# vaenyr/stable-diffusion-on-device

Hardware: AMD Instinct MI355X
Metric: images/sec + per-UNet-step ms, SD v1.4 512x512 20-step PLMS, 1/2/4/8 MI355X (higher is better)
Workload: dtype f16; 1 GPU; SD v1.4 txt2img 512x512, 20-step PLMS (21 UNet evals, batch 2 = cond+uncond per image), CLIP encode + VAE decode + uint8, guidance 7.5; images_per_gpu=1, global_batch=1, parallelism=dp1 (image shards, 1 RCCL broadcast), hip_graph=True, trajectory_graph=True, decode_overlaps_next_sampling=False

## Files before the change

include/sdod_engine.h:

```cpp
#ifndef SDOD_ENGINE_H
#define SDOD_ENGINE_H

#include <stddef.h>
#include <stdint.h>

#ifndef SDOD_API
#define SDOD_API
#endif

#ifdef __cplusplus
extern "C" {
#endif

enum sdod_graph_kind { SDOD_GRAPH_UNET = 0, SDOD_GRAPH_VAE_DECODER = 1, SDOD_GRAPH_TEXT_ENCODER = 2, SDOD_GRAPH_TEMB = 3,
                       SDOD_GRAPH_VAE_ENCODER = 4, SDOD_GRAPH_VAE_ENCODER_MASKED = 5, SDOD_GRAPH_ADAPTER = 6, SDOD_GRAPH_UPSCALER = 7 };

typedef struct sdod_model_config {
    int latent_channels;
    int latent_h;
    int latent_w;
    int model_channels;
    int context_dim;
    int context_len;
    int num_heads;
    int head_dim;
    int vocab_size;
    int text_layers;
    int text_heads;
    int vae_channels;
    int linear_proj;
    int text_arch;
    int weight_quant;
    int concat_channels;
} sdod_model_config;

SDOD_API void sdod_model_config_sd14(sdod_model_config* cfg);
SDOD_API void sdod_model_config_sd21(sdod_model_config* cfg);

SDOD_API int sdod_graph_create(void** graph, int kind, const sdod_model_config* cfg, int batch);
typedef struct sdod_adapter_config {
    int adapter_reps;
    int adapter_hint_channels;
    int adapter_res_blocks;
} sdod_adapter_config;
SDOD_API int sdod_graph_create_ex(void** graph, int kind, const sdod_model_config* cfg, const sdod_adapter_config* adapter, int batch);
SDOD_API int sdod_graph_create_wrap(void** graph, int kind, const sdod_model_config* cfg, const sdod_adapter_config* adapter, int wrap,
                                    int batch);
typedef struct sdod_upscaler_config {
    int num_blocks;
    int in_h;
    int in_w;
} sdod_upscaler_config;
SDOD_API int sdod_graph_create_upscaler(void** graph, const sdod_upscaler_config* cfg, int batch);
SDOD_API int sdod_graph_destroy(void* graph);

SDOD_API int sdod_graph_num_params(void* graph);
SDOD_API int sdod_graph_param_info(void* graph, int index, const char** name, int* ndim, int64_t shape[4]);
SDOD_API int sdod_graph_set_param(void* graph, const char* name, const void* data, int dtype, const int64_t* shape, int ndim);
SDOD_API int sdod_graph_param_device(void* graph, const char* name, void** device_ptr, size_t* bytes);
SDOD_API int sdod_graph_load_file(void* graph, const char* path, const char* prefix);
SDOD_API int sdod_graph_finalize(void* graph);
SDOD_API int sdod_graph_io(void* graph, int is_output, int index, void** device_ptr, size_t* bytes);
enum sdod_exec_flags { SDOD_EXEC_HIP_GRAPH = 1, SDOD_EXEC_STATIC_UNCHANGED = 2 };
SDOD_API int sdod_graph_execute(void* graph, void* stream, int flags);
SDOD_API int sdod_graph_check(void* graph);
SDOD_API int sdod_graph_num_ops(void* graph);
SDOD_API int sdod_graph_op_info(void* graph, int index, const char** label, double* flops, double* bytes);
SDOD_API int sdod_graph_op_detail(void* graph, int index, const char** detail);
SDOD_API int sdod_graph_profile(void* graph, void* stream, int iters, float* ms_out, int n);
SDOD_API int sdod_graph_stats(void* graph, size_t* weight_bytes, size_t* arena_bytes, int* num_launches, double* flops);
SDOD_API int sdod_graph_tune_info(void* graph, int* from_table, int* tuned_in_process, char* table_path, int cap);

SDOD_API int sdod_graph_keep_base(void* graph);
SDOD_API int sdod_graph_base_bytes(void* graph, size_t* bytes);
typedef struct {
    const char* name;
    const void* up;
    const void* down;
    int dtype;
    int rank;
    float scale;
} sdod_lora_entry;
SDOD_API int sdod_graph_set_loras(void* graph, const sdod_lora_entry* entries, int count, void* stream);

#ifdef __cplusplus
}
#endif
#endif
```

include/sdod_hip.h:

```cpp
#ifndef SDOD_HIP_H
#define SDOD_HIP_H

#include <stddef.h>
#include <stdint.h>

#ifndef SDOD_API
#define SDOD_API
#endif

#ifdef __cplusplus
extern "C" {
#endif

enum sdod_act { SDOD_ACT_NONE = 0, SDOD_ACT_SILU = 1, SDOD_ACT_GELU = 2, SDOD_ACT_QUICK_GELU = 3, SDOD_ACT_RELU = 4 };
enum sdod_dtype { SDOD_F16 = 0, SDOD_F32 = 1, SDOD_U8Q = 2, SDOD_BF16 = 3  };
enum sdod_a_mode { SDOD_A_ROWS = 0, SDOD_A_CONV3X3 = 1  };

typedef struct sdod_gemm_desc {
    const void* a;
    const void* a2;
    const void* w;
    const void* bias;
    const void* row_bias;
    const void* residual;
// ... 33 lines not shown
    int vec_img_stride;
    int softmax_cols;
    int pad_mode;
} sdod_gemm_desc;

SDOD_API int sdod_gemm_f16(const sdod_gemm_desc* d, void* stream);
SDOD_API int sdod_gemm_fixup(const sdod_gemm_desc* d);
SDOD_API size_t sdod_gemm_fixup_counters(void);
SDOD_API size_t sdod_gemm_workspace_bytes(const sdod_gemm_desc* d);
SDOD_API int sdod_gemm_plan(const sdod_gemm_desc* d, int* tile, int* splits);
SDOD_API int sdod_gemm_halo_ok(const sdod_gemm_desc* d, int tile);
SDOD_API int sdod_gemm_panel_ok(const sdod_gemm_desc* d, int tile);
SDOD_API int sdod_gemm_xcd_panels(const sdod_gemm_desc* d);
SDOD_API int sdod_gemm_num_tiles(void);
SDOD_API int sdod_gemm_tile_shape(int tile, int* bm, int* bn, int* lds_dma);
SDOD_API int sdod_gemm_tile_info(int tile, int out[7]);
SDOD_API int sdod_gemm_time(const sdod_gemm_desc* d, void* stream, int iters, float* ms_avg);
SDOD_API int sdod_gemm_time_cold(const sdod_gemm_desc* d, void* stream, int iters, void* scratch, size_t scratch_bytes, float* ms_avg,
                                float* ms_min );

SDOD_API size_t sdod_group_norm_workspace_bytes(int n, int groups);
SDOD_API int sdod_group_norm_layout(int n, int groups, size_t* sync_off, size_t* partial_off, size_t* stats_off, size_t* shift_off,
                                    size_t* end_off);
SDOD_API int sdod_group_norm_status(void);
SDOD_API int sdod_group_norm_clear_error(void);
SDOD_API int sdod_group_norm_launches(int hw, int c, int groups, int dtype);
SDOD_API int sdod_group_norm_path(int n, int hw, int c0, int c1, int groups, int dtype);
SDOD_API int sdod_group_norm_nhwc(const void* x, const void* x2, void* y, const float* weight, const float* bias,
                                  int n, int hw, int c0, int c1, int groups, float eps, int silu, int dtype,
                                  void* workspace, void* stream);

SDOD_API size_t sdod_group_norm_nchw_workspace_bytes(int n, int groups);
SDOD_API int sdod_group_norm_nchw(const void* x, void* y, const float* weight, const float* bias, int n, int c, long long spatial,
                                  int groups, float eps, int silu, int dtype, void* workspace, void* stream);

typedef struct sdod_gn_reduce {
    const void* partial;
    int splits;
    size_t slab_floats;
    const void* bias;
    const void* bias2;
    const void* row_bias;
    int ld_row_bias;
    const void* residual;
    int ldr;
    void* x_out;
    float alpha;
    int act;
    int M, N;
} sdod_gn_reduce;
SDOD_API int sdod_gemm_reduce_info(const sdod_gemm_desc* d, sdod_gn_reduce* out);
SDOD_API int sdod_group_norm_reduce_ok(int hw, int c0, int c1, int groups);
SDOD_API int sdod_group_norm_reduce_nhwc(const sdod_gn_reduce* red, const void* x2, void* y, const float* weight,
                                         const float* bias, int n, int hw, int c0, int c1, int groups, float eps, int silu,
                                         void* stream);

SDOD_API int sdod_ln_fold_f16(void* w, int n, int k, int ldw, const float* gamma, const float* beta, const float* bias_in,
                              float* s_out, float* t_out, void* stream);
SDOD_API int sdod_compose_linear_f16(const void* p, int ldp, const void* w, int ldw, void* c, int ldc, int n_out, int n_mid, int k,
                                     const float* bias_w, const float* bias_p, float* bias_out, void* stream);
SDOD_API int sdod_lora_merge_f16(void* w, int n, int k, int ldw, const void* up, const void* down, int rank, float scale,
                                 int conv_cin, int geglu, void* stream);
SDOD_API int sdod_layer_norm_f16(const void* x, void* y, const float* weight, const float* bias, int m, int c,
                                 float eps, void* stream);

SDOD_API int sdod_attention_f16(const void* q, const void* k, const void* v, void* out, int batch, int heads,
                                int lq, int lk, int d, int ldq, int ldk, int ldv, int ldo, float scale, int causal,
                                void* stream);

SDOD_API int sdod_xattn_fold_f16(const void* kv, int ld_kv, int k_off, int v_off, int n_img, int L, const void* wq, int ldq,
                                 const void* sq, const void* tq, const void* wo, int ldwo, int heads, int d, float scale, void* w1,
                                 void* s1, void* t1, void* w2, void* stream);

SDOD_API int sdod_softmax_rows_f16(const void* x, void* y, int m, int n, void* stream);

SDOD_API int sdod_geglu_f16(const void* x, void* y, int m, int c, void* stream);
SDOD_API int sdod_act_f16(const void* x, void* y, size_t n, int act, void* stream);
SDOD_API int sdod_add_f16(const void* a, const void* b, void* y, size_t n, void* stream);
SDOD_API int sdod_concat_channels_f16(const void* a, const void* b, void* y, size_t rows, int c0, int c1, void* stream);
SDOD_API int sdod_pixel_unshuffle_u8_f16(const uint8_t* img, void* y, int n, int h, int w, int ch, int factor, void* stream);
SDOD_API int sdod_avg_pool2_f16(const void* x, void* y, int n, int h, int w, int c, void* stream);
SDOD_API int sdod_adapter_stage_f16(const void* src, void* dst, size_t count, float weight, void* stream);
SDOD_API int sdod_add_feature_f16(void* h, const void* f, size_t per_copy, int reps, void* stream);
SDOD_API int sdod_im2col3x3_small_f16(const void* x, void* y, int n_img, int h, int w, int c, int kpad, void* stream);
SDOD_API int sdod_im2col3x3_small_wrap_f16(const void* x, void* y, int n_img, int h, int w, int c, int kpad, int wrap, void* stream);
SDOD_API int sdod_latent_im2col_f16(const float* x, void* y, int n_img, int h, int w, int c, int kpad, float scale, void* stream);

SDOD_API int sdod_conv_in_f16(const float* x, const void* w, const float* bias, void* y, int n_img, int h, int wd, int c, int cout,
                              float scale, void* stream);
SDOD_API int sdod_conv_in_wrap_f16(const float* x, const void* w, const float* bias, void* y, int n_img, int h, int wd, int c, int cout,
                                   float scale, int wrap, void* stream);
SDOD_API int sdod_image_conv_in_f16(const uint8_t* img, const void* w, const float* bias, void* y, int n_img, int h, int wd, int cout,
                                    void* stream);
SDOD_API int sdod_conv_in_cat_f16(const float* x, const float* cond, const void* w, const float* bias, void* y, int n_img, int h, int wd,
                                  int c, int c_cond, int cout, void* stream);
SDOD_API int sdod_masked_image_conv_in_f16(const uint8_t* img, const uint8_t* mask, const void* w, const float* bias, void* y, int n_img,
                                           int h, int wd, int cout, void* stream);
SDOD_API int sdod_image_conv_in_unit_f16(const uint8_t* img, const void* w, const float* bias, void* y, void* y2, int ld2, int n_img, int h,
                                         int wd, int cout, void* stream);

typedef struct sdod_dense_conv_desc {
    const void* in;
    const void* w;
    const float* bias;
    void* out;
    const void* res1;
    const void* res2;
    int ld_in, ld_out, ld_res1, ld_res2;
    int out_col;
    int cin, cout;
    int n, h, w_in;
    int upsample;
    float alpha, slope, c1;
} sdod_dense_conv_desc;
SDOD_API int sdod_dense_conv3x3_f16(const sdod_dense_conv_desc* d, void* stream);
SDOD_API int sdod_dense_conv3x3_ok(const sdod_dense_conv_desc* d);

SDOD_API int sdod_inpaint_cond_f32(const float* moments, const uint8_t* mask_u8, const float* n1, float* cond, int n, int c, int h_lat,
                                   int w_lat, int factor, int reps, uint64_t seed, uint64_t image_index0, void* stream);
SDOD_API int sdod_encode_latent_f32(const float* moments, const float* n1, const float* n2, float* x, float* z0, int n, int c, int hw,
                                    float sqrt_at, float sqrt_one_minus_at, uint64_t seed, uint64_t image_index0, void* stream);
SDOD_API int sdod_latent_resize_f32(const float* src, float* dst, int n, int c, int h_in, int w_in, int h_out, int w_out, int mode, float a,
                                    float b, const float* noise, uint64_t seed, uint64_t image_index0, void* stream);
SDOD_API int sdod_latent_resize_taps(int mode, int n_in, int n_out, int32_t* idx, float* w);
SDOD_API int sdod_nchw_f32_to_nhwc_f16(const float* x, void* y, int n, int c, int hw, float scale, void* stream);
SDOD_API int sdod_latent_prep_f16(const float* x, const float* w, const float* b, void* y, int n, int c, int hw,
                                  float scale, void* stream);
SDOD_API int sdod_nhwc_f16_to_nchw_f32(const void* x, float* y, int n, int c, int hw, void* stream);
SDOD_API int sdod_embedding_f16(const int32_t* ids, const void* table, const void* pos, void* y, int rows, int seq,
                                int c, void* stream);
SDOD_API int sdod_context_assemble_f16(const void* enc, const float* w, void* out, int P, int K, int T, int D, void* stream);
SDOD_API int sdod_timestep_features_f16(const float* t, void* y, int n, int dim, void* stream);

SDOD_API int sdod_stage_unet_inputs(const float* x, float* x_dst, size_t lat_count, int reps, const void* temb_row,
                                    void* temb_dst, size_t temb_width, int temb_reps, void* stream);
SDOD_API int sdod_randn_f32(float* out, uint32_t* words_out, size_t count, uint64_t seed, uint64_t stream_id, void* stream);

SDOD_API int sdod_cfg_combine(const void* eps_nhwc, float* e_out, int n, int c, int hw, float guidance,
                              int uncond_first, int mode, void* stream);
SDOD_API int sdod_dpm_update(float* x, const float* eps, float* y_prev, size_t count, int order, float sigma_s,
                             float alpha_s, float sigma_ratio, float c_prev, float c_cur, void* stream);
SDOD_API int sdod_ddim_step_f32(float* x, const float* e, size_t count, float sqrt_one_minus_at, float sqrt_at,
                                float sqrt_a_prev, float dir_coef, void* stream);
SDOD_API int sdod_lincomb4_f32(float* out, const float* e0, const float* e1, const float* e2, const float* e3,
                               float c0, float c1, float c2, float c3, float div, size_t count, void* stream);

typedef struct sdod_plms_update_args {
    const void* eps_nhwc;
    float* e_out;
    float* x;
    const float* old1; const float* old2; const float* old3;
    float* x_stage;
    const void* temb_row;
    void* temb_dst;
    int n, c, hw, uncond_first, mode, v_pred, stage_reps, temb_width, temb_reps;
    float guidance, vc0, vc1, c0, c1, c2, c3, div, sqrt_one_minus_at, sqrt_at, sqrt_a_prev, dir_coef;
} sdod_plms_update_args;
SDOD_API int sdod_plms_update(const sdod_plms_update_args* a, void* stream);

typedef struct sdod_dpm_step_args {
    const void* eps_nhwc;
    float* e_out;
    float* x;
    float* y_prev;
    float* x_stage;
    const void* temb_row;
// ... 49 lines not shown
```

stable-diffusion-on-device_amd/csrc/elementwise.hip:

```cpp
#include "common.h"
#include <atomic>
#include <cmath>
#include "sdod_hip.h"
#include "host_util.h"

#pragma clang fp contract(off)

namespace {

SDOD_DEVICE float mul_rn(float a, float b) { return a * b; }
SDOD_DEVICE float add_rn(float a, float b) { return a + b; }
SDOD_DEVICE float sub_rn(float a, float b) { return a - b; }
SDOD_DEVICE float div_rn(float a, float b) { return a / b; }

inline int grid_for(size_t work, int block = 256) {
    size_t b = (work + block - 1) / block;
    if (b > 2048) b = 2048;
    if (b < 1) b = 1;
    return (int)b;
}

#define GRID_STRIDE(i, n) \
    for (size_t i = (size_t)blockIdx.x * blockDim.x + threadIdx.x; i < (n); i += (size_t)gridDim.x * blockDim.x)

// ... 14 lines not shown

__global__ void act_kernel(const f16* x, f16* y, size_t n8, int act) {
    GRID_STRIDE(i, n8) {
        const f16x8 a = ldg8(x + i * 8);
        f16x8 o;
#pragma unroll
        for (int e = 0; e < 8; ++e) o[e] = (f16)apply_act((float)a[e], act);
        stg8(y + i * 8, o);
    }
}

__global__ void add_kernel(const f16* a, const f16* b, f16* y, size_t n8) {
    GRID_STRIDE(i, n8) {
        const f16x8 u = ldg8(a + i * 8), v = ldg8(b + i * 8);
        f16x8 o;
#pragma unroll
        for (int e = 0; e < 8; ++e) o[e] = (f16)((float)u[e] + (float)v[e]);
        stg8(y + i * 8, o);
    }
}

__global__ void relu_kernel(const f16* x, f16* y, size_t n8) {
    GRID_STRIDE(i, n8) {
        const f16x8 a = ldg8(x + i * 8);
        f16x8 o;
#pragma unroll
        for (int e = 0; e < 8; ++e) o[e] = a[e] < (f16)0.0f ? (f16)0.0f : a[e];
        stg8(y + i * 8, o);
    }
}

__global__ void pixel_unshuffle_kernel(const uint8_t* img, f16* y, size_t total, int h, int w, int ch) {
    GRID_STRIDE(t, total) {
        const int dy = (int)(t & 7);
        const size_t q = t >> 3;
        const int c = (int)(q % ch);
        const size_t pix = q / ch;
        const size_t j = pix % w, bi = pix / w;
        const uint8_t* src = img + ((bi * 8 + dy) * ((size_t)w * 8) + j * 8) * ch + c;
        f16x8 o;
#pragma unroll
        for (int dx = 0; dx < 8; ++dx) o[dx] = (f16)div_rn((float)src[(size_t)dx * ch], 255.0f);
        stg8(y + t * 8, o);
    }
}

__global__ void avg_pool2_kernel(const f16* x, f16* y, size_t total, int ho, int wo, int c) {
    const int cp = c / 8;
    GRID_STRIDE(t, total) {
        const int c8 = (int)(t % cp) * 8;
        const size_t pix = t / cp;
        const size_t j = pix % wo, bi = pix / wo;
        const f16* r0 = x + ((bi * 2) * ((size_t)wo * 2) + j * 2) * c + c8;
        const f16* r1 = r0 + (size_t)wo * 2 * c;
        const f16x8 a = ldg8(r0), b = ldg8(r0 + c), cc = ldg8(r1), d = ldg8(r1 + c);
        f16x8 o;
#pragma unroll
        for (int e = 0; e < 8; ++e)
            o[e] = (f16)mul_rn(add_rn(add_rn((float)a[e], (float)b[e]), add_rn((float)cc[e], (float)d[e])), 0.25f);
        stg8(y + pix * c + c8, o);
    }
}

__global__ void adapter_stage_kernel(const f16* src, f16* dst, size_t n8, float weight) {
    GRID_STRIDE(i, n8) {
        const f16x8 a = ldg8(src + i * 8);
        f16x8 o;
#pragma unroll
        for (int e = 0; e < 8; ++e) o[e] = (f16)mul_rn(weight, (float)a[e]);
        stg8(dst + i * 8, o);
    }
}

__global__ void add_feature_kernel(f16* h, const f16* f, size_t n8, size_t per_copy, int reps) {
    GRID_STRIDE(i, n8) {
        const f16x8 v = ldg8(f + i * 8);
        for (int r = 0; r < reps; ++r) {
            f16* p = h + (size_t)r * per_copy + i * 8;
            const f16x8 u = ldg8(p);
            f16x8 o;
#pragma unroll
            for (int e = 0; e < 8; ++e) o[e] = (f16)add_rn((float)u[e], (float)v[e]);
            stg8(p, o);
        }
    }
}

__global__ void concat_kernel(const f16* a, const f16* b, f16* y, size_t rows, int c0, int c1) {
    const int cp = (c0 + c1) / 8, cp0 = c0 / 8;
    const size_t total = rows * cp;
    GRID_STRIDE(i, total) {
        const size_t r = i / cp;
        const int ch = (int)(i - r * cp);
        const f16x8 v = ch < cp0 ? ldg8(a + r * c0 + ch * 8) : ldg8(b + r * c1 + (ch - cp0) * 8);
        stg8(y + r * (c0 + c1) + ch * 8, v);
    }
}

SDOD_DEVICE int wrap1(int v, int n) {
    v += v < 0 ? n : 0;
    return v - (v >= n ? n : 0);
}

__global__ void im2col_small_kernel(const f16* x, f16* y, int n_img, int h, int w, int c, int kpad, int wrap) {
    const size_t total = (size_t)n_img * h * w * kpad;
    GRID_STRIDE(i, total) {
        const size_t row = i / kpad;
        const int k = (int)(i - row * kpad);
        f16 v = (f16)0.f;
        if (k < 9 * c) {
            const int tap = k / c, ch = k - tap * c;
            const int r = tap / 3, s = tap - r * 3;
            const int img = (int)(row / ((size_t)h * w));
            const int rem = (int)(row - (size_t)img * h * w);
            const int oy = rem / w, ox = rem - oy * w;
            int yy = oy + r - 1, xx = ox + s - 1;
            if (wrap & 2) yy = wrap1(yy, h);
            if (wrap & 1) xx = wrap1(xx, w);
            if (yy >= 0 && yy < h && xx >= 0 && xx < w) v = x[(((size_t)img * h + yy) * w + xx) * c + ch];
        }
        y[i] = v;
    }
}

__global__ void latent_im2col_kernel(const float* x, f16* y, int n_img, int h, int w, int c, int kpad, float scale) {
    const int kp8 = kpad / 8;
    const size_t total = (size_t)n_img * h * w * kp8;
    GRID_STRIDE(i, total) {
        const size_t row = i / kp8;
        const int k0 = (int)(i - row * kp8) * 8;
        const int img = (int)(row / ((size_t)h * w));
        const int rem = (int)(row - (size_t)img * h * w);
        const int oy = rem / w, ox = rem - oy * w;
        f16x8 v;
#pragma unroll
        for (int e = 0; e < 8; ++e) {
            const int k = k0 + e;
            float f = 0.f;
            if (k < 9 * c) {
                const int tap = k / c, ch = k - tap * c;
                const int r = tap / 3, s2 = tap - r * 3;
                const int yy = oy + r - 1, xx = ox + s2 - 1;
                if (yy >= 0 && yy < h && xx >= 0 && xx < w) f = 0.f + x[(((size_t)img * c + ch) * h + yy) * w + xx] * scale;
            }
            v[e] = (f16)f;
        }
        *reinterpret_cast<f16x8*>(y + row * kpad + k0) = v;
    }
}

struct LatentSrc {
    const float* x;
    float scale;
    SDOD_DEVICE float at(int img, int ch, int yy, int xx, int c, int h, int wd) const {
        return 0.f + x[((size_t)img * c + ch) * h * wd + (size_t)yy * wd + xx] * scale;
    }
};
struct ImageU8Src {
    const uint8_t* img;
    SDOD_DEVICE float at(int img_i, int ch, int yy, int xx, int c, int h, int wd) const {
        return 2.0f * ((float)img[(((size_t)img_i * h + yy) * wd + xx) * c + ch] / 255.0f) - 1.0f;
    }
};
struct ImageU8UnitSrc {
    const uint8_t* img;
    f16* y2;
// ... 703 lines not shown
            }
            if (a.den_prev) *reinterpret_cast<f32x4*>(a.den_prev + o) = den;
        } else {
#pragma unroll
            for (int q = 0; q < 4; ++q) out[q] = div_rn(mul_rn(a.a, xv[q]), 1.0f);
        }
        *reinterpret_cast<f32x4*>(a.x + o) = out;
        if (a.x_stage) {
            f32x4 st;
#pragma unroll
            for (int q = 0; q < 4; ++q) st[q] = mul_rn(a.stage_scale, out[q]);
            stage_latent(a.x_stage, a.stage_reps, lat, o, st);
        }
    }
}

#define LAUNCH(kernel, work, st, ...)                                                            \
    do {                                                                                         \
        SDOD_LAUNCH(kernel, dim3(grid_for(work)), dim3(256), 0, (hipStream_t)(st), __VA_ARGS__); \
        SDOD_HIP_CHECK(hipGetLastError());                                                       \
    } while (0)

extern "C" int sdod_geglu_f16(const void* x, void* y, int m, int c, void* stream) {
    SDOD_TRY
    SDOD_REQUIRE(x && y && m > 0 && c > 0 && c % 8 == 0, "bad argument");
    LAUNCH(geglu_kernel, (size_t)m * (c / 8), stream, (const f16*)x, (f16*)y, m, c);
    return 0;
    SDOD_CATCH
}

extern "C" int sdod_act_f16(const void* x, void* y, size_t n, int act, void* stream) {
    SDOD_TRY
    SDOD_REQUIRE(x && y && n > 0 && n % 8 == 0, "bad argument (count must be a multiple of 8)");
    if (act == ACT_RELU) LAUNCH(relu_kernel, n / 8, stream, (const f16*)x, (f16*)y, n / 8);
    else LAUNCH(act_kernel, n / 8, stream, (const f16*)x, (f16*)y, n / 8, act);
    return 0;
    SDOD_CATCH
}

extern "C" int sdod_pixel_unshuffle_u8_f16(const uint8_t* img, void* y, int n, int h, int w, int ch, int factor, void* stream) {
    SDOD_TRY
    SDOD_REQUIRE(img && y && n > 0 && h > 0 && w > 0, "bad argument");
    SDOD_REQUIRE(factor == 8, "the adapter's input is unshuffled by 8: factor must be 8");
    SDOD_REQUIRE(ch == 1 || ch == 3, "ch must be 1 or 3");
    SDOD_REQUIRE(((uintptr_t)y & 15) == 0, "misaligned pointer (y: 16 bytes)");
    const size_t total = (size_t)n * h * w * ch * 8;
    LAUNCH(pixel_unshuffle_kernel, total, stream, img, (f16*)y, total, h, w, ch);
    return 0;
    SDOD_CATCH
}

extern "C" int sdod_avg_pool2_f16(const void* x, void* y, int n, int h, int w, int c, void* stream) {
    SDOD_TRY
    SDOD_REQUIRE(x && y && n > 0 && h > 0 && w > 0 && c > 0, "bad argument");
    SDOD_REQUIRE(h % 2 == 0 && w % 2 == 0, "h and w must be even");
    SDOD_REQUIRE(c % 8 == 0, "c must be a multiple of 8");
    SDOD_REQUIRE((((uintptr_t)x | (uintptr_t)y) & 15) == 0, "misaligned pointer (16 bytes)");
    const size_t total = (size_t)n * (h / 2) * (w / 2) * (c / 8);
    LAUNCH(avg_pool2_kernel, total, stream, (const f16*)x, (f16*)y, total, h / 2, w / 2, c);
    return 0;
    SDOD_CATCH
}

extern "C" int sdod_adapter_stage_f16(const void* src, void* dst, size_t count, float weight, void* stream) {
    SDOD_TRY
    SDOD_REQUIRE(src && dst && count > 0 && count % 8 == 0, "bad argument (count must be a multiple of 8)");
    SDOD_REQUIRE(std::isfinite(weight), "weight must be finite");
    SDOD_REQUIRE((((uintptr_t)src | (uintptr_t)dst) & 15) == 0, "misaligned pointer (16 bytes)");
    LAUNCH(adapter_stage_kernel, count / 8, stream, (const f16*)src, (f16*)dst, count / 8, weight);
    return 0;
    SDOD_CATCH
}

extern "C" int sdod_add_feature_f16(void* h, const void* f, size_t per_copy, int reps, void* stream) {
    SDOD_TRY
    SDOD_REQUIRE(h && f && per_copy > 0 && per_copy % 8 == 0, "bad argument (per_copy must be a multiple of 8)");
    SDOD_REQUIRE(reps == 1 || reps == 2, "reps must be 1 or 2 (the guidance copies)");
    SDOD_REQUIRE((((uintptr_t)h | (uintptr_t)f) & 15) == 0, "misaligned pointer (16 bytes)");
    LAUNCH(add_feature_kernel, per_copy / 8, stream, (f16*)h, (const f16*)f, per_copy / 8, per_copy, reps);
    return 0;
    SDOD_CATCH
}

extern "C" int sdod_add_f16(const void* a, const void* b, void* y, size_t n, void* stream) {
    SDOD_TRY
    SDOD_REQUIRE(a && b && y && n > 0 && n % 8 == 0, "bad argument (count must be a multiple of 8)");
    LAUNCH(add_kernel, n / 8, stream, (const f16*)a, (const f16*)b, (f16*)y, n / 8);
    return 0;
    SDOD_CATCH
}

extern "C" int sdod_concat_channels_f16(const void* a, const void* b, void* y, size_t rows, int c0, int c1, void* stream) {
    SDOD_TRY
    SDOD_REQUIRE(a && b && y && rows > 0 && c0 > 0 && c1 > 0 && c0 % 8 == 0 && c1 % 8 == 0, "bad argument");
    LAUNCH(concat_kernel, rows * ((c0 + c1) / 8), stream, (const f16*)a, (const f16*)b, (f16*)y, rows, c0, c1);
    return 0;
    SDOD_CATCH
}

extern "C" int sdod_im2col3x3_small_wrap_f16(const void* x, void* y, int n_img, int h, int w, int c, int kpad, int wrap, void* stream) {
    SDOD_TRY
    SDOD_REQUIRE(x && y && n_img > 0 && h > 0 && w > 0 && c > 0 && kpad >= 9 * c, "bad argument");
    SDOD_REQUIRE(wrap >= 0 && wrap <= 3, "wrap must be 0 .. 3 (bit 0 = x, bit 1 = y)");
    LAUNCH(im2col_small_kernel, (size_t)n_img * h * w * kpad, stream, (const f16*)x, (f16*)y, n_img, h, w, c, kpad, wrap);
    return 0;
    SDOD_CATCH
}

extern "C" int sdod_im2col3x3_small_f16(const void* x, void* y, int n_img, int h, int w, int c, int kpad, void* stream) {
    return sdod_im2col3x3_small_wrap_f16(x, y, n_img, h, w, c, kpad, 0, stream);
}

extern "C" int sdod_latent_im2col_f16(const float* x, void* y, int n_img, int h, int w, int c, int kpad, float scale, void* stream) {
    SDOD_TRY
    SDOD_REQUIRE(x && y && n_img > 0 && h > 0 && w > 0 && c > 0 && kpad >= 9 * c && kpad % 8 == 0 && ((uintptr_t)y & 15) == 0, "bad argument");
    LAUNCH(latent_im2col_kernel, (size_t)n_img * h * w * (kpad / 8), stream, x, (f16*)y, n_img, h, w, c, kpad, scale);
    return 0;
    SDOD_CATCH
}

template <typename Src, int KS = 2>
void launch_conv_in(const Src src, const void* w, const float* bias, void* y, int n_img, int h, int wd, int c, int cout, hipStream_t st, int wrap = 0) {
    const long long M = (long long)n_img * h * wd;
    const dim3 grid((unsigned)((M + 31) / 32));
    switch (cout / 64) {
    case 1: SDOD_LAUNCH((conv_in_kernel<1, Src, KS>), grid, dim3(256), 0, st, src, (const f16*)w, bias, (f16*)y, n_img, h, wd, c, wrap); break;
    case 2: SDOD_LAUNCH((conv_in_kernel<2, Src, KS>), grid, dim3(256), 0, st, src, (const f16*)w, bias, (f16*)y, n_img, h, wd, c, wrap); break;
    case 4: SDOD_LAUNCH((conv_in_kernel<4, Src, KS>), grid, dim3(256), 0, st, src, (const f16*)w, bias, (f16*)y, n_img, h, wd, c, wrap); break;
    default: SDOD_LAUNCH((conv_in_kernel<5, Src, KS>), grid, dim3(256), 0, st, src, (const f16*)w, bias, (f16*)y, n_img, h, wd, c, wrap); break;
    }
    SDOD_HIP_CHECK(hipGetLastError());
}

extern "C" int sdod_conv_in_wrap_f16(const float* x, const void* w, const float* bias, void* y, int n_img, int h, int wd, int c, int cout,
                                     float scale, int wrap, void* stream) {
    SDOD_TRY
    SDOD_REQUIRE(wrap >= 0 && wrap <= 3, "wrap must be 0 .. 3 (bit 0 = x, bit 1 = y)");
    SDOD_REQUIRE(x && w && y && n_img > 0 && h > 0 && wd > 0 && c > 0 && 9 * c <= 64, "bad argument (9 * Cin must fit the 64-deep K slab)");
    SDOD_REQUIRE(cout == 320 || cout == 256 || cout == 128 || cout == 64, "Cout must be 64, 128, 256 or 320");
    SDOD_REQUIRE((((uintptr_t)w | (uintptr_t)bias) & 15) == 0 && ((uintptr_t)y & 7) == 0, "misaligned pointer");
    launch_conv_in(LatentSrc{x, scale}, w, bias, y, n_img, h, wd, c, cout, (hipStream_t)stream, wrap);
    return 0;
    SDOD_CATCH
}

extern "C" int sdod_conv_in_f16(const float* x, const void* w, const float* bias, void* y, int n_img, int h, int wd, int c, int cout,
                                float scale, void* stream) {
    return sdod_conv_in_wrap_f16(x, w, bias, y, n_img, h, wd, c, cout, scale, 0, stream);
}

extern "C" int sdod_image_conv_in_f16(const uint8_t* img, const void* w, const float* bias, void* y, int n_img, int h, int wd, int cout,
                                      void* stream) {
    SDOD_TRY
    SDOD_REQUIRE(img && w && y && n_img > 0 && h > 0 && wd > 0, "bad argument");
    SDOD_REQUIRE(cout == 320 || cout == 256 || cout == 128 || cout == 64, "Cout must be 64, 128, 256 or 320");
    SDOD_REQUIRE((((uintptr_t)w | (uintptr_t)bias) & 15) == 0 && ((uintptr_t)y & 7) == 0, "misaligned pointer");
    launch_conv_in(ImageU8Src{img}, w, bias, y, n_img, h, wd, 3, cout, (hipStream_t)stream);
    return 0;
    SDOD_CATCH
}

extern "C" int sdod_image_conv_in_unit_f16(const uint8_t* img, const void* w, const float* bias, void* y, void* y2, int ld2, int n_img, int h,
                                           int wd, int cout, void* stream) {
    SDOD_TRY
    SDOD_REQUIRE(img && w && y && n_img > 0 && h > 0 && wd > 0, "bad argument");
    SDOD_REQUIRE(cout == 320 || cout == 256 || cout == 128 || cout == 64, "Cout must be 64, 128, 256 or 320");
// ... 330 lines not shown
```

stable-diffusion-on-device_amd/csrc/engine.h:

```cpp
#pragma once
#include <hip/hip_runtime.h>

#include <cstdint>
#include <functional>
#include <map>
#include <string>
#include <unordered_map>
#include <vector>

#include "host_util.h"
#include "sdod_engine.h"
#include "sdod_hip.h"

namespace sdod {

typedef _Float16 f16;

enum ParamKind {
    PK_CONV3,
    PK_CONV3_SMALL,
    PK_CONV1,
    PK_LINEAR,
    PK_EMBED,
    PK_VEC,
    PK_MAT_F32,
    PK_LINEAR_GEGLU,
    PK_VEC_GEGLU,
};

inline int small_k(int64_t cin) { return 9 * cin <= 64 ? 64 : 128; }

struct Param {
    std::string name;
    std::vector<int64_t> shape;
    ParamKind kind;
    int group = -1;
    int ld = 0;
    int col_off = 0;
    int owner = -1;
    size_t dev_bytes = 0;
    char* dev = nullptr;
    bool set = false;
    bool quant = false;
    size_t qrow = 0;
};

struct Act {
    f16* p = nullptr;
    int n = 0, h = 0, w = 0, c = 0;
    int rows() const { return n * h * w; }
    size_t numel() const { return (size_t)rows() * c; }
};

struct IoSlot {
    void* ptr = nullptr;
    size_t bytes = 0;
};

class Graph {
public:
    Graph(int kind, const sdod_model_config& cfg, int batch, const sdod_adapter_config& acfg = sdod_adapter_config{0, 0, 0}, int wrap = 0,
          const sdod_upscaler_config& ucfg = sdod_upscaler_config{0, 0, 0});
    ~Graph();
    Graph(const Graph&) = delete;

    int num_params() const { return (int)params_.size(); }
    const Param& param(int i) const { return params_.at(i); }
    void set_param(const std::string& name, const void* data, int dtype, const int64_t* shape, int ndim);
    void load_file(const std::string& path, const std::string& prefix);
    void finalize();
    void keep_base();
    size_t base_bytes() const { return base_copy_ ? weight_bytes_ : 0; }
    void set_loras(const sdod_lora_entry* entries, int count, hipStream_t st);
    void execute(hipStream_t st, bool use_hip_graph, bool skip_static = false);
    void check_health() const;
    IoSlot io(bool output, int index) const;
    void stats(size_t* wbytes, size_t* abytes, int* launches, double* flops) const;

private:
    enum Mode { DECLARE, DRY, REAL };
    int kind_;
    sdod_model_config cfg_;
    sdod_adapter_config acfg_;
    sdod_upscaler_config ucfg_;
    int batch_;
    int wrap_ = 0;
    Mode mode_ = DECLARE;
    bool finalized_ = false;

    std::vector<Param> params_;
    std::unordered_map<std::string, int> pindex_;
    std::vector<std::vector<int>> groups_;
    std::unordered_map<std::string, int> gindex_;
    char* weight_base_ = nullptr;
    size_t weight_bytes_ = 0;
    float* qscale_ = nullptr;
    float* qoff_ = nullptr;
    size_t qrows_ = 0;
    bool quant_mode() const { return cfg_.weight_quant != 0 && (kind_ == SDOD_GRAPH_UNET || kind_ == SDOD_GRAPH_TEMB); }
    static constexpr int kQuantAutoMaxRows = 128;
    bool quant_decl_ = false;
    void quant_rows(int rows) { quant_decl_ = quant_mode() && (cfg_.weight_quant == 1 || rows <= kQuantAutoMaxRows); }
    void quant_global() { quant_decl_ = quant_mode(); }
    const float* qscale_of(int w) const { return params_[w].quant ? qscale_ + params_[w].qrow : nullptr; }
    const float* qoff_of(int w) const { return params_[w].quant ? qoff_ + params_[w].qrow : nullptr; }
    int P(const std::string& name, std::vector<int64_t> shape, ParamKind kind, const std::string& group = "");
    int Pc(const std::string& name, std::vector<int64_t> shape, ParamKind kind, int ld, int col_off, int owner);
    template <typename T>
    const T* W(int idx) const { return reinterpret_cast<const T*>(params_[idx].dev); }
    void allocate_weights();

    char* arena_base_ = nullptr;
    size_t arena_cap_ = 0, arena_high_ = 0;
    std::map<size_t, size_t> free_;
    std::map<size_t, size_t> used_;
    void arena_reset();
    f16* alloc(size_t halves);
    void release(const void* p);
    Act act(int n, int h, int w, int c);
    void release(const Act& a) { release(a.p); }

    char* ws_ = nullptr;
    size_t ws_bytes_ = 0, ws_need_ = 0;
    char* gn_ws_ = nullptr;
    size_t gn_ws_bytes_ = 0, gn_ws_need_ = 0;

    std::vector<IoSlot> inputs_, outputs_;
    void* io_alloc(std::vector<IoSlot>& v, size_t bytes);

    struct Op {
        std::function<void(hipStream_t)> fn;
        std::string label;
        double flops = 0;
        double bytes = 0;
        std::string detail;
        const void* pf_ptr = nullptr;
        size_t pf_bytes = 0;
    };
    std::vector<Op> ops_;
    std::vector<Op> static_ops_;
    bool to_static_ = false;
    double flops_ = 0;
    hipGraphExec_t graph_exec_ = nullptr;
    hipGraph_t hip_graph_ = nullptr;
    hipStream_t capture_stream_ = nullptr;
    unsigned* fix_counters_ = nullptr;
    hipStream_t side_stream_ = nullptr;
    std::vector<hipEvent_t> pf_events_;
    void run_ops(hipStream_t st);
    int eager_runs_ = 0;
    int tune_hits_ = 0, tune_misses_ = 0;

    void build();
    void build_unet();
    void build_vae();
    void build_vae_encoder(bool masked);
    void build_clip();
    void build_temb();
    void build_adapter();
    void build_upscaler();

    struct GemmOpt {
        int bias = -1;
        const float* bias_raw = nullptr;
        f16* out = nullptr;
        const f16* row_bias = nullptr;
        int ld_row_bias = 0, rows_per_img = 0;
        const f16* residual = nullptr;
        int act = 0;
        float alpha = 1.0f;
        bool bias_on_m = false;
        int lda = 0, ldo = 0;
        int ldr = 0;
        bool geglu = false;
        const Act* tail0 = nullptr;
        const Act* tail1 = nullptr;
        int bias2 = -1;
        int ln_w = -1, ln_b = -1;
        const float* wq_scale = nullptr;
        const float* wq_off = nullptr;
        const float* ln_s_raw = nullptr;
        int w_img_stride = 0, vec_img_stride = 0;
        int softmax_cols = 0;
        int pad_mode = 0;
        int split_k = 0;
    };
    struct LnVecs { float* s; float* t; };
    LnVecs ln_fold_vectors(f16* w, int N, int K, int ldw, int ln_w, int ln_b, const float* bias);
    struct FoldJob {
        f16* w; int n, k, ldw;
        const float *gamma, *beta, *bias_in;
        float *s, *t;
    };
    std::vector<FoldJob> fold_jobs_;
    struct ComposeJob {
        f16* c; const f16* p; int ld, n_out, n_mid, k;
        const float *bias_w, *bias_p;
        float* bias_out;
    };
    std::vector<ComposeJob> compose_jobs_;
    void run_folds(hipStream_t st);
    bool keep_base_ = false;
    char* base_copy_ = nullptr;
    bool static_stale_ = false;
    std::vector<void*> derived_;
    void emit_gemm(sdod_gemm_desc d);
    void linear(const f16* x, int rows, int K, int w, int N, f16* out, const GemmOpt& o);
    void linear_raw(const f16* x, int rows, int K, const f16* w, int ldw, int N, f16* out, const GemmOpt& o);
    Act conv(const Act& x, const Act* x2, int w, int cout, int ksize, int stride, bool upsample, const GemmOpt& o);
    Act group_norm(const Act& x, const Act* x2, int gw, int gb, float eps, bool silu);
    Act layer_norm(const Act& x, int lw, int lb, float eps);
    void dense_conv(sdod_dense_conv_desc d, int w, int bias);
    void attention(const f16* q, const f16* k, const f16* v, f16* out, int B, int heads, int lq, int lk, int d, int ldq,
                   int ldk, int ldv, int ldo, bool causal);

    Act res_block(const std::string& pfx, const Act& x, const Act* x2, int cout, const f16* emb_all, int emb_ld, int& emb_off);
    std::vector<Op>& sink() { return to_static_ ? static_ops_ : ops_; }
    struct PendingReduce {
        bool active = false;
        sdod_gemm_desc d{};
        double bytes = 0;
        std::string detail;
    } pending_;
    void flush_pending();
    std::vector<const void*> parked_;
    void release_after_consumer(const Act& a) { parked_.push_back(a.p); }
    void drain_parked() {
        for (const void* p : parked_) release(p);
        parked_.clear();
    }
    void settle() {
        flush_pending();
        drain_parked();
    }
    Act spatial_transformer(const std::string& pfx, const Act& x, const Act& ctx);
    Act vae_res_block(const std::string& pfx, const Act& x, int cout);
    Act vae_attn_block(const std::string& pfx, const Act& x);
    int emb_total_ = 0;
    int kv_total_ = 0;
    f16* kv_all_ = nullptr;
    int kv_off_ = 0;
    std::vector<std::pair<std::string, int>> unet_res_blocks() const;
    const char* group_base(const std::string& group) const;
    int group_first(const std::string& group) const;
    void emit(std::function<void(hipStream_t)> fn, const char* label = "elementwise", double flops = 0, double bytes = 0) {
        settle();
        if (mode_ == REAL) sink().push_back(Op{std::move(fn), label, flops, bytes, ""});
    }

public:
    int tune_hits() const { return tune_hits_; }
    int tune_misses() const { return tune_misses_; }
    int num_ops() const { return (int)ops_.size(); }
    const Op& op(int i) const { return ops_.at(i); }
    void profile(hipStream_t st, int iters, float* ms, int n);
};

}
```

stable-diffusion-on-device_amd/csrc/engine.hip:

```cpp
#include "engine.h"

#include <cstdio>

#include <dlfcn.h>
#include <fcntl.h>
#include <sys/mman.h>
#include <sys/stat.h>
#include <unistd.h>

#include <algorithm>
#include <cstdlib>
#include <cstring>
#include <map>
#include <mutex>
#include <thread>

namespace sdod {

static inline size_t align_up(size_t v, size_t a) { return (v + a - 1) / a * a; }

static void check_rc(int rc) {
    if (rc != 0) throw Error(rc, get_last_error());
}

template <typename F>
static void parallel_for(int64_t n, F&& fn) {
    int nt = (int)std::min<int64_t>(n, std::max(1u, std::min(16u, std::thread::hardware_concurrency())));
    if (nt <= 1) {
        fn(0, n);
        return;
    }
    std::vector<std::thread> th;
    const int64_t per = (n + nt - 1) / nt;
    for (int t = 0; t < nt; ++t) {
        const int64_t b = t * per, e = std::min(n, b + per);
        if (b < e) th.emplace_back([=, &fn]() { fn(b, e); });
    }
    for (auto& t : th) t.join();
}

Graph::Graph(int kind, const sdod_model_config& cfg, int batch, const sdod_adapter_config& acfg, int wrap, const sdod_upscaler_config& ucfg)
    : kind_(kind), cfg_(cfg), acfg_(acfg), ucfg_(ucfg), batch_(batch), wrap_(wrap) {
    SDOD_REQUIRE(kind >= SDOD_GRAPH_UNET && kind <= SDOD_GRAPH_UPSCALER, "unknown graph kind");
    if (kind == SDOD_GRAPH_UPSCALER) {
        SDOD_REQUIRE(ucfg.num_blocks != 0 || ucfg.in_h != 0 || ucfg.in_w != 0, "the UPSCALER graph is created by sdod_graph_create_upscaler");
        SDOD_REQUIRE(ucfg.num_blocks >= 1 && ucfg.num_blocks <= 23, "num_blocks must be in [1, 23]");
        SDOD_REQUIRE(ucfg.in_h >= 8 && ucfg.in_h <= 1024 && ucfg.in_h % 8 == 0 && ucfg.in_w >= 8 && ucfg.in_w <= 1024 && ucfg.in_w % 8 == 0,
                     "in_h and in_w must be multiples of 8 in [8, 1024]");
        cfg_.weight_quant = 0;
    } else {
        SDOD_REQUIRE(ucfg.num_blocks == 0 && ucfg.in_h == 0 && ucfg.in_w == 0, "an upscaler configuration needs kind SDOD_GRAPH_UPSCALER");
    }
    SDOD_REQUIRE(batch > 0 && batch <= 64, "batch must be in [1, 64]");
    SDOD_REQUIRE(cfg.model_channels > 0 && cfg.model_channels % 64 == 0, "model_channels must be a multiple of 64");
    SDOD_REQUIRE(cfg.context_dim % 64 == 0, "context_dim must be a multiple of 64");
    SDOD_REQUIRE(cfg.context_len >= 1 && cfg.context_len <= 4096, "context_len must be in [1, 4096]");
    SDOD_REQUIRE(cfg.concat_channels >= 0, "concat_channels must not be negative");
    SDOD_REQUIRE(acfg.adapter_reps >= 0 && acfg.adapter_reps <= 2, "adapter_reps must be 0, 1 or 2");
    SDOD_REQUIRE(wrap >= 0 && wrap <= 3, "wrap must be 0 .. 3 (bit 0 = x, bit 1 = y)");
    if (wrap != 0)
        SDOD_REQUIRE((kind == SDOD_GRAPH_UNET || kind == SDOD_GRAPH_VAE_DECODER) && cfg.concat_channels == 0,
                     "wrap applies to the UNET (without concat_channels) and VAE_DECODER graphs only");
    if (kind == SDOD_GRAPH_UNET && acfg.adapter_reps > 0)
        SDOD_REQUIRE(batch % acfg.adapter_reps == 0, "adapter_reps must divide the batch");
    if (kind == SDOD_GRAPH_ADAPTER) {
        SDOD_REQUIRE(acfg.adapter_hint_channels == 1 || acfg.adapter_hint_channels == 3, "adapter_hint_channels must be 1 or 3");
        SDOD_REQUIRE(acfg.adapter_res_blocks >= 0 && acfg.adapter_res_blocks <= 8, "adapter_res_blocks must be in [1, 8] (0 = 2)");
        cfg_.weight_quant = 0;
    }
    mode_ = DECLARE;
    arena_reset();
    build();
}

Graph::~Graph() {
    if (graph_exec_) (void)hipGraphExecDestroy(graph_exec_);
    if (capture_stream_) (void)hipStreamDestroy(capture_stream_);
    if (side_stream_) (void)hipStreamDestroy(side_stream_);
    (void)hipFree(fix_counters_);
    for (hipEvent_t e : pf_events_) (void)hipEventDestroy(e);
    if (hip_graph_) (void)hipGraphDestroy(hip_graph_);
    for (auto& s : inputs_) (void)hipFree(s.ptr);
    for (auto& s : outputs_) (void)hipFree(s.ptr);
    (void)hipFree(weight_base_);
    (void)hipFree(base_copy_);
    (void)hipFree(qscale_);
    (void)hipFree(qoff_);
    (void)hipFree(arena_base_);
    (void)hipFree(ws_);
    (void)hipFree(gn_ws_);
    (void)hipFree(kv_all_);
    for (void* d : derived_) (void)hipFree(d);
}

static size_t param_dev_bytes(const Param& p) {
    const auto& s = p.shape;
    if (p.quant) return (size_t)s[0] * s[1] * (p.kind == PK_CONV3 ? 9 : 1);
    switch (p.kind) {
    case PK_CONV3: return (size_t)s[0] * s[1] * 9 * sizeof(f16);
    case PK_CONV3_SMALL: return (size_t)s[0] * small_k(s[1]) * sizeof(f16);
    case PK_CONV1:
    case PK_LINEAR:
    case PK_LINEAR_GEGLU:
    case PK_EMBED: return (size_t)s[0] * s[1] * sizeof(f16);
    case PK_VEC:
    case PK_VEC_GEGLU: return (size_t)s[0] * sizeof(float);
    case PK_MAT_F32: {
        size_t n = 1;
        for (auto d : s) n *= (size_t)d;
        return n * sizeof(float);
    }
    }
    return 0;
}

int Graph::P(const std::string& name, std::vector<int64_t> shape, ParamKind kind, const std::string& group) {
    if (mode_ != DECLARE) {
        auto it = pindex_.find(name);
        if (it == pindex_.end()) throw Error(INTERNAL_ERROR, "parameter not declared: " + name);
        return it->second;
    }
    if (pindex_.count(name)) throw Error(INTERNAL_ERROR, "duplicate parameter: " + name);
    Param p;
    p.name = name;
    p.shape = std::move(shape);
    p.kind = kind;
    p.quant = quant_decl_ && (kind == PK_CONV3 || kind == PK_CONV1 || kind == PK_LINEAR || kind == PK_LINEAR_GEGLU);
    p.dev_bytes = param_dev_bytes(p);
    if (!group.empty()) {
        auto it = gindex_.find(group);
        if (it == gindex_.end()) {
            gindex_[group] = (int)groups_.size();
            groups_.emplace_back();
            it = gindex_.find(group);
        }
        p.group = it->second;
        groups_[p.group].push_back((int)params_.size());
    }
    pindex_[name] = (int)params_.size();
    params_.push_back(std::move(p));
    return (int)params_.size() - 1;
}

int Graph::Pc(const std::string& name, std::vector<int64_t> shape, ParamKind kind, int ld, int col_off, int owner) {
    const int idx = P(name, std::move(shape), kind);
    if (mode_ == DECLARE) {
        Param& p = params_[idx];
// ... 1043 lines not shown
            }
            samples[i].push_back(tot);
        }
    }
    for (size_t i = 0; i < ops_.size(); ++i) {
        std::sort(samples[i].begin(), samples[i].end());
        const size_t k = samples[i].size();
        ms[i] = k == 0 ? 0.f : (k & 1) ? samples[i][k / 2] : 0.5f * (samples[i][k / 2 - 1] + samples[i][k / 2]);
    }
    ++eager_runs_;
}

void Graph::stats(size_t* wbytes, size_t* abytes, int* launches, double* flops) const {
    if (wbytes) *wbytes = weight_bytes_;
    if (abytes) *abytes = arena_cap_;
    if (launches) *launches = (int)ops_.size();
    if (flops) *flops = flops_;
}

}

using sdod::Graph;

extern "C" void sdod_model_config_sd14(sdod_model_config* cfg) {
    if (!cfg) return;
    cfg->latent_channels = 4;
    cfg->latent_h = 64;
    cfg->latent_w = 64;
    cfg->model_channels = 320;
    cfg->context_dim = 768;
    cfg->context_len = 77;
    cfg->num_heads = 8;
    cfg->head_dim = 0;
    cfg->vocab_size = 49408;
    cfg->text_layers = 12;
    cfg->text_heads = 12;
    cfg->vae_channels = 128;
    cfg->linear_proj = 0;
    cfg->text_arch = 0;
    cfg->concat_channels = 0;
}

extern "C" void sdod_model_config_sd21(sdod_model_config* cfg) {
    if (!cfg) return;
    sdod_model_config_sd14(cfg);
    cfg->latent_h = cfg->latent_w = 96;
    cfg->context_dim = 1024;
    cfg->num_heads = 0;
    cfg->head_dim = 64;
    cfg->linear_proj = 1;
    cfg->text_arch = 1;
    cfg->text_layers = 23;
    cfg->text_heads = 16;
}

extern "C" int sdod_graph_create(void** graph, int kind, const sdod_model_config* cfg, int batch) {
    SDOD_TRY
    SDOD_REQUIRE(graph != nullptr && cfg != nullptr, "null argument");
    *graph = nullptr;
    *graph = new Graph(kind, *cfg, batch);
    return 0;
    SDOD_CATCH
}

extern "C" int sdod_graph_create_ex(void** graph, int kind, const sdod_model_config* cfg, const sdod_adapter_config* adapter, int batch) {
    SDOD_TRY
    SDOD_REQUIRE(graph != nullptr && cfg != nullptr, "null argument");
    *graph = nullptr;
    *graph = new Graph(kind, *cfg, batch, adapter ? *adapter : sdod_adapter_config{0, 0, 0});
    return 0;
    SDOD_CATCH
}

extern "C" int sdod_graph_create_wrap(void** graph, int kind, const sdod_model_config* cfg, const sdod_adapter_config* adapter, int wrap,
                                      int batch) {
    SDOD_TRY
    SDOD_REQUIRE(graph != nullptr && cfg != nullptr, "null argument");
    *graph = nullptr;
    *graph = new Graph(kind, *cfg, batch, adapter ? *adapter : sdod_adapter_config{0, 0, 0}, wrap);
    return 0;
    SDOD_CATCH
}

extern "C" int sdod_graph_create_upscaler(void** graph, const sdod_upscaler_config* ucfg, int batch) {
    SDOD_TRY
    SDOD_REQUIRE(graph != nullptr, "null argument");
    *graph = nullptr;
    SDOD_REQUIRE(ucfg != nullptr, "null upscaler configuration");
    sdod_model_config cfg{};
    sdod_model_config_sd14(&cfg);
    *graph = new Graph(SDOD_GRAPH_UPSCALER, cfg, batch, sdod_adapter_config{0, 0, 0}, 0, *ucfg);
    return 0;
    SDOD_CATCH
}

extern "C" int sdod_graph_destroy(void* graph) {
    SDOD_TRY
    delete static_cast<Graph*>(graph);
    return 0;
    SDOD_CATCH
}

extern "C" int sdod_graph_num_params(void* graph) { return graph ? static_cast<Graph*>(graph)->num_params() : 0; }

extern "C" int sdod_graph_param_info(void* graph, int index, const char** name, int* ndim, int64_t shape[4]) {
    SDOD_TRY
    SDOD_REQUIRE(graph != nullptr, "null graph");
    auto* g = static_cast<Graph*>(graph);
    SDOD_REQUIRE(index >= 0 && index < g->num_params(), "parameter index out of range");
    const sdod::Param& p = g->param(index);
    if (name) *name = p.name.c_str();
    if (ndim) *ndim = (int)p.shape.size();
    if (shape)
        for (size_t i = 0; i < 4; ++i) shape[i] = i < p.shape.size() ? p.shape[i] : 1;
    return 0;
    SDOD_CATCH
}

extern "C" int sdod_graph_set_param(void* graph, const char* name, const void* data, int dtype, const int64_t* shape, int ndim) {
    SDOD_TRY
    SDOD_REQUIRE(graph && name && shape, "null argument");
    static_cast<Graph*>(graph)->set_param(name, data, dtype, shape, ndim);
    return 0;
    SDOD_CATCH
}

extern "C" int sdod_graph_load_file(void* graph, const char* path, const char* prefix) {
    SDOD_TRY
    SDOD_REQUIRE(graph && path, "null argument");
    static_cast<Graph*>(graph)->load_file(path, prefix ? prefix : "");
    return 0;
    SDOD_CATCH
}

extern "C" int sdod_graph_finalize(void* graph) {
    SDOD_TRY
    SDOD_REQUIRE(graph != nullptr, "null graph");
    static_cast<Graph*>(graph)->finalize();
    return 0;
    SDOD_CATCH
}

extern "C" int sdod_graph_io(void* graph, int is_output, int index, void** device_ptr, size_t* bytes) {
    SDOD_TRY
    SDOD_REQUIRE(graph != nullptr, "null graph");
    const sdod::IoSlot s = static_cast<Graph*>(graph)->io(is_output != 0, index);
    if (device_ptr) *device_ptr = s.ptr;
    if (bytes) *bytes = s.bytes;
    return 0;
    SDOD_CATCH
}

extern "C" int sdod_graph_param_device(void* graph, const char* name, void** device_ptr, size_t* bytes) {
    SDOD_TRY
    SDOD_REQUIRE(graph != nullptr && name != nullptr, "null argument");
    Graph* g = static_cast<Graph*>(graph);
    for (int i = 0; i < g->num_params(); ++i) {
        const sdod::Param& p = g->param(i);
        if (p.name != name) continue;
        SDOD_REQUIRE(p.dev != nullptr && p.set, "parameter '" + p.name + "' has not been set");
        if (device_ptr) *device_ptr = p.dev;
        if (bytes) *bytes = p.dev_bytes;
        return 0;
    }
    SDOD_REQUIRE(false, std::string("unknown parameter '") + name + "'");
    return 0;
// ... 99 lines not shown
```

stable-diffusion-on-device_amd/csrc/graphs.hip:

```cpp
#include "engine.h"

namespace sdod {

static void check_rc2(int rc) {
    if (rc != 0) throw Error(rc, get_last_error());
}

int Graph::group_first(const std::string& group) const {
    auto it = gindex_.find(group);
    if (it == gindex_.end()) throw Error(INTERNAL_ERROR, "unknown parameter group " + group);
    return groups_[it->second].front();
}

const char* Graph::group_base(const std::string& group) const {
    auto it = gindex_.find(group);
    if (it == gindex_.end()) throw Error(INTERNAL_ERROR, "unknown parameter group " + group);
    return params_[groups_[it->second].front()].dev;
}

Act Graph::res_block(const std::string& pfx, const Act& x, const Act* x2, int cout, const f16* emb_all, int emb_ld, int& emb_off) {
    const int cin = x.c + (x2 ? x2->c : 0);
    quant_rows(x.rows());
    const int n1w = P(pfx + ".in_layers.0.weight", {cin}, PK_VEC), n1b = P(pfx + ".in_layers.0.bias", {cin}, PK_VEC);
    const int c1w = P(pfx + ".in_layers.2.weight", {cout, cin, 3, 3}, PK_CONV3), c1b = P(pfx + ".in_layers.2.bias", {cout}, PK_VEC);
    const int n2w = P(pfx + ".out_layers.0.weight", {cout}, PK_VEC), n2b = P(pfx + ".out_layers.0.bias", {cout}, PK_VEC);
    int c2w, skw = -1, skb = -1;
    const bool fuse_skip = !quant_decl_;
    if (cin != cout && !fuse_skip) {
        c2w = P(pfx + ".out_layers.3.weight", {cout, cout, 3, 3}, PK_CONV3);
        skw = P(pfx + ".skip_connection.weight", {cout, cin, 1, 1}, PK_CONV1);
        skb = P(pfx + ".skip_connection.bias", {cout}, PK_VEC);
    } else if (cin != cout) {
        const int ld = 9 * cout + cin;
        c2w = Pc(pfx + ".out_layers.3.weight", {cout, cout, 3, 3}, PK_CONV3, ld, 0, -1);
        skw = Pc(pfx + ".skip_connection.weight", {cout, cin, 1, 1}, PK_CONV1, ld, 9 * cout, c2w);
        skb = P(pfx + ".skip_connection.bias", {cout}, PK_VEC);
    } else {
        c2w = P(pfx + ".out_layers.3.weight", {cout, cout, 3, 3}, PK_CONV3);
    }
    const int c2b = P(pfx + ".out_layers.3.bias", {cout}, PK_VEC);
    (void)skw;
    const int my_off = emb_off;
    emb_off += cout;

    Act g1 = group_norm(x, x2, n1w, n1b, 1e-5f, true);
    GemmOpt o1;
    o1.bias = c1b;
    o1.row_bias = emb_all ? emb_all + my_off : nullptr;
    o1.ld_row_bias = emb_ld;
    o1.rows_per_img = x.h * x.w;
    Act h = conv(g1, nullptr, c1w, cout, 3, 1, false, o1);
    release(g1);
    Act g2 = group_norm(h, nullptr, n2w, n2b, 1e-5f, true);
    release(h);
    GemmOpt o2;
    o2.bias = c2b;
    Act sk;
    if (cin != cout && !fuse_skip) {
        GemmOpt os;
        os.bias = skb;
        sk = conv(x, x2, skw, cout, 1, 1, false, os);
        o2.residual = sk.p;
    } else if (cin != cout) {
        o2.tail0 = &x;
        o2.tail1 = x2;
        o2.bias2 = skb;
    } else {
        if (x2) throw Error(INTERNAL_ERROR, "identity skip with a concatenated input");
        o2.residual = x.p;
    }
    Act out = conv(g2, nullptr, c2w, cout, 3, 1, false, o2);
    release(g2);
    if (sk.p) release_after_consumer(sk);
    return out;
}

Act Graph::spatial_transformer(const std::string& pfx, const Act& x, const Act& ctx) {
    const int C = x.c, cd = ctx.c;
    const int heads = cfg_.num_heads > 0 ? cfg_.num_heads : C / cfg_.head_dim;
    const int d = C / heads;
    const int rows = x.rows(), L = x.h * x.w, B = x.n;
    const std::string tb = pfx + ".transformer_blocks.0";
    quant_rows(rows);
    const bool quant_block = quant_decl_;
    const int nw = P(pfx + ".norm.weight", {C}, PK_VEC), nb = P(pfx + ".norm.bias", {C}, PK_VEC);
    const bool lin = cfg_.linear_proj != 0;
    const int piw = lin ? P(pfx + ".proj_in.weight", {C, C}, PK_LINEAR) : P(pfx + ".proj_in.weight", {C, C, 1, 1}, PK_CONV1);
    const int pib = P(pfx + ".proj_in.bias", {C}, PK_VEC);
    const int l1w = P(tb + ".norm1.weight", {C}, PK_VEC), l1b = P(tb + ".norm1.bias", {C}, PK_VEC);
    const std::string gq = tb + ".attn1.qkv";
    P(tb + ".attn1.to_q.weight", {C, C}, PK_LINEAR, gq);
    P(tb + ".attn1.to_k.weight", {C, C}, PK_LINEAR, gq);
    P(tb + ".attn1.to_v.weight", {C, C}, PK_LINEAR, gq);
    const int o1w = P(tb + ".attn1.to_out.0.weight", {C, C}, PK_LINEAR), o1b = P(tb + ".attn1.to_out.0.bias", {C}, PK_VEC);
    const int l2w = P(tb + ".norm2.weight", {C}, PK_VEC), l2b = P(tb + ".norm2.bias", {C}, PK_VEC);
    const int q2w = P(tb + ".attn2.to_q.weight", {C, C}, PK_LINEAR);
    quant_global();
    P(tb + ".attn2.to_k.weight", {C, cd}, PK_LINEAR, "attn2_kv_all");
    P(tb + ".attn2.to_v.weight", {C, cd}, PK_LINEAR, "attn2_kv_all");
    quant_decl_ = quant_block;
    const int my_kv = kv_off_;
    kv_off_ += 2 * C;
    const int o2w = P(tb + ".attn2.to_out.0.weight", {C, C}, PK_LINEAR), o2b = P(tb + ".attn2.to_out.0.bias", {C}, PK_VEC);
    const int l3w = P(tb + ".norm3.weight", {C}, PK_VEC), l3b = P(tb + ".norm3.bias", {C}, PK_VEC);
    const int f1w = P(tb + ".ff.net.0.proj.weight", {8 * C, C}, PK_LINEAR_GEGLU), f1b = P(tb + ".ff.net.0.proj.bias", {8 * C}, PK_VEC_GEGLU);
    static const bool compose_on = [] { const char* e = std::getenv("SDOD_COMPOSE"); return !(e && e[0] == '0'); }();
    const bool compose = compose_on && !quant_block;
    int f2w, pow_;
    if (compose) {
        f2w = Pc(tb + ".ff.net.2.weight", {C, 4 * C}, PK_LINEAR, 5 * C, 0, -1);
        pow_ = lin ? Pc(pfx + ".proj_out.weight", {C, C}, PK_LINEAR, 5 * C, 4 * C, f2w)
                   : Pc(pfx + ".proj_out.weight", {C, C, 1, 1}, PK_CONV1, 5 * C, 4 * C, f2w);
    } else {
        f2w = P(tb + ".ff.net.2.weight", {C, 4 * C}, PK_LINEAR);
        pow_ = lin ? P(pfx + ".proj_out.weight", {C, C}, PK_LINEAR) : P(pfx + ".proj_out.weight", {C, C, 1, 1}, PK_CONV1);
    }
    const int f2b = P(tb + ".ff.net.2.bias", {C}, PK_VEC);
    const int pob = P(pfx + ".proj_out.bias", {C}, PK_VEC);
    if (mode_ == DECLARE) return act(x.n, x.h, x.w, C);

    Act g = group_norm(x, nullptr, nw, nb, 1e-6f, false);
    Act t0 = act(B, 1, L, C);
    { GemmOpt o; o.bias = pib; linear(g.p, rows, C, piw, C, t0.p, o); }
    release(g);
    const bool fold = !quant_block;
    auto normed = [&](const Act& src, int lw, int lb) -> Act { return layer_norm(src, lw, lb, 1e-5f); };
    f16* qkv = alloc((size_t)rows * 3 * C);
    if (fold) {
        GemmOpt o; o.ln_w = l1w; o.ln_b = l1b;
        linear_raw(t0.p, rows, C, reinterpret_cast<const f16*>(group_base(gq)), C, 3 * C, qkv, o);
    } else {
        Act nrm = normed(t0, l1w, l1b);
        GemmOpt o; o.wq_scale = qscale_of(group_first(gq)); o.wq_off = qoff_of(group_first(gq));
        linear_raw(nrm.p, rows, C, reinterpret_cast<const f16*>(group_base(gq)), C, 3 * C, qkv, o);
        release(nrm);
    }
    f16* a1 = alloc((size_t)rows * C);
    attention(qkv, qkv + C, qkv + 2 * C, a1, B, heads, L, L, d, 3 * C, 3 * C, 3 * C, C, false);
    release(qkv);
    Act t1 = act(B, 1, L, C);
    { GemmOpt o; o.bias = o1b; o.residual = t0.p; linear(a1, rows, C, o1w, C, t1.p, o); }
    release(a1); release(t0);
    static const bool xfold_on = [] { const char* e = std::getenv("SDOD_XATTN_FOLD"); return !(e && e[0] == '0'); }();
    const int NK = heads * 80;
    const bool xfold = xfold_on && fold && ctx.w <= 80 && NK % 320 == 0 && L % 32 == 0 && d <= 160 && d % 4 == 0;
    if (xfold) {
        f16 *w1 = nullptr, *w2 = nullptr;
        float *s1 = nullptr, *t1v = nullptr;
        f16* wq = reinterpret_cast<f16*>(params_[q2w].dev);
        const f16* wo = reinterpret_cast<const f16*>(params_[o2w].dev);
        if (mode_ == REAL) {
            SDOD_HIP_CHECK(hipMalloc((void**)&w1, (size_t)B * NK * C * sizeof(f16)));
            SDOD_HIP_CHECK(hipMalloc((void**)&w2, (size_t)B * NK * C * sizeof(f16)));
            SDOD_HIP_CHECK(hipMalloc((void**)&s1, (size_t)B * NK * sizeof(float)));
            SDOD_HIP_CHECK(hipMalloc((void**)&t1v, (size_t)B * NK * sizeof(float)));
            derived_.push_back(w1); derived_.push_back(w2); derived_.push_back(s1); derived_.push_back(t1v);
            const LnVecs qv = ln_fold_vectors(wq, C, C, C, l2w, l2b, nullptr);
            const f16* kvp = kv_all_;
            const int ldkv = kv_total_, koff = my_kv, Lk = ctx.w, hh = heads, dd = d;
            const float scale = 1.0f / sqrtf((float)d);
            to_static_ = true;
            sink().push_back(Op{[=](hipStream_t st) {
                check_rc2(sdod_xattn_fold_f16(kvp, ldkv, koff, koff + C, B, Lk, wq, C, qv.s, qv.t, wo, C, hh, dd, scale, w1, s1, t1v, w2, st));
            }, "xattn_fold", 4.0 * B * NK * (double)C * d, 4.0 * B * NK * C * 2, "C" + std::to_string(C) + " d" + std::to_string(d)});
            to_static_ = false;
        }
        const f16* w1p = mode_ == REAL ? w1 : wq;
        const f16* w2p = mode_ == REAL ? w2 : wq;
        f16* pb = alloc((size_t)rows * NK);
        { GemmOpt o; o.ln_s_raw = mode_ == REAL ? s1 : reinterpret_cast<const float*>(wq); o.bias_raw = mode_ == REAL ? t1v : reinterpret_cast<const float*>(wq);
          o.w_img_stride = NK * C; o.vec_img_stride = NK; o.softmax_cols = 80; o.rows_per_img = L;
          linear_raw(t1.p, rows, C, w1p, C, NK, pb, o); }
        GemmOpt o2;
        o2.bias = o2b; o2.residual = t1.p; o2.w_img_stride = C * NK; o2.rows_per_img = L;
        if (compose) {
            f16* cat = alloc((size_t)rows * 5 * C);
            f16* t2c = cat + 4 * C;
            o2.ldr = C; o2.ldo = 5 * C;
            linear_raw(pb, rows, NK, w2p, NK, C, t2c, o2);
            release(pb); release(t1);
            { GemmOpt o; o.bias = f1b; o.geglu = true; o.ln_w = l3w; o.ln_b = l3b; o.lda = 5 * C; o.ldo = 5 * C; linear(t2c, rows, C, f1w, 8 * C, cat, o); }
            float* bc = nullptr;
            if (mode_ == REAL) {
                SDOD_HIP_CHECK(hipMalloc((void**)&bc, (size_t)C * sizeof(float)));
                derived_.push_back(bc);
                f16* wc = reinterpret_cast<f16*>(params_[f2w].dev);
                compose_jobs_.push_back(ComposeJob{wc, wc + 4 * C, 5 * C, C, C, 4 * C, W<float>(f2b), W<float>(pob), bc});
            }
            Act out = act(x.n, x.h, x.w, C);
            { GemmOpt o; o.bias_raw = mode_ == REAL ? bc : reinterpret_cast<const float*>(params_[f2w].dev); o.residual = x.p;
              linear_raw(cat, rows, 5 * C, reinterpret_cast<const f16*>(params_[f2w].dev), 5 * C, C, out.p, o); }
            release(cat);
            return out;
        }
        Act t2 = act(B, 1, L, C);
        linear_raw(pb, rows, NK, w2p, NK, C, t2.p, o2);
        release(pb); release(t1);
        f16* gg = alloc((size_t)rows * 4 * C);
        { GemmOpt o; o.bias = f1b; o.geglu = true; o.ln_w = l3w; o.ln_b = l3b; linear(t2.p, rows, C, f1w, 8 * C, gg, o); }
        Act t3 = act(B, 1, L, C);
        { GemmOpt o; o.bias = f2b; o.residual = t2.p; linear(gg, rows, 4 * C, f2w, C, t3.p, o); }
        release(gg); release(t2);
        Act out = act(x.n, x.h, x.w, C);
        { GemmOpt o; o.bias = pob; o.residual = x.p; linear(t3.p, rows, C, pow_, C, out.p, o); }
        release(t3);
        return out;
    }
    f16* q2 = alloc((size_t)rows * C);
    if (fold) {
        GemmOpt o; o.ln_w = l2w; o.ln_b = l2b; linear(t1.p, rows, C, q2w, C, q2, o);
    } else {
        Act nrm = normed(t1, l2w, l2b);
        linear(nrm.p, rows, C, q2w, C, q2, GemmOpt{});
        release(nrm);
    }
    const int Lk = ctx.w;
    const f16* kv = kv_all_ + my_kv;
    f16* a2 = alloc((size_t)rows * C);
    attention(q2, kv, kv + C, a2, B, heads, L, Lk, d, C, kv_total_, kv_total_, C, false);
    release(q2);
    if (compose) {
        f16* cat = alloc((size_t)rows * 5 * C);
        f16* t2c = cat + 4 * C;
        { GemmOpt o; o.bias = o2b; o.residual = t1.p; o.ldr = C; o.ldo = 5 * C; linear(a2, rows, C, o2w, C, t2c, o); }
        release(a2); release(t1);
        { GemmOpt o; o.bias = f1b; o.geglu = true; o.ln_w = l3w; o.ln_b = l3b; o.lda = 5 * C; o.ldo = 5 * C; linear(t2c, rows, C, f1w, 8 * C, cat, o); }
        float* bc = nullptr;
        if (mode_ == REAL) {
            SDOD_HIP_CHECK(hipMalloc((void**)&bc, (size_t)C * sizeof(float)));
            derived_.push_back(bc);
            f16* wc = reinterpret_cast<f16*>(params_[f2w].dev);
            compose_jobs_.push_back(ComposeJob{wc, wc + 4 * C, 5 * C, C, C, 4 * C, W<float>(f2b), W<float>(pob), bc});
        }
        Act out = act(x.n, x.h, x.w, C);
        { GemmOpt o; o.bias_raw = mode_ == REAL ? bc : reinterpret_cast<const float*>(params_[f2w].dev); o.residual = x.p;
          linear_raw(cat, rows, 5 * C, reinterpret_cast<const f16*>(params_[f2w].dev), 5 * C, C, out.p, o); }
        release(cat);
        return out;
    }
    Act t2 = act(B, 1, L, C);
    { GemmOpt o; o.bias = o2b; o.residual = t1.p; linear(a2, rows, C, o2w, C, t2.p, o); }
    release(a2); release(t1);
    f16* gg = alloc((size_t)rows * 4 * C);
    if (fold) {
        GemmOpt o; o.bias = f1b; o.geglu = true; o.ln_w = l3w; o.ln_b = l3b; linear(t2.p, rows, C, f1w, 8 * C, gg, o);
    } else {
        Act nrm = normed(t2, l3w, l3b);
        GemmOpt o; o.bias = f1b; o.geglu = true; linear(nrm.p, rows, C, f1w, 8 * C, gg, o);
        release(nrm);
    }
    Act t3 = act(B, 1, L, C);
    { GemmOpt o; o.bias = f2b; o.residual = t2.p; linear(gg, rows, 4 * C, f2w, C, t3.p, o); }
    release(gg); release(t2);
    Act out = act(x.n, x.h, x.w, C);
    { GemmOpt o; o.bias = pob; o.residual = x.p; linear(t3.p, rows, C, pow_, C, out.p, o); }
    release(t3);
    return out;
}

void Graph::build_unet() {
    const int B = batch_, H = cfg_.latent_h, Wd = cfg_.latent_w, LC = cfg_.latent_channels;
    const int MC = cfg_.model_channels, EC = 4 * MC, cd = cfg_.context_dim, CL = cfg_.context_len;
    const int CC = cfg_.concat_channels, CI = LC + CC;
    SDOD_REQUIRE(LC * 9 <= 64, "latent_channels too large for the small-Cin path");
    SDOD_REQUIRE(H >= 8 && Wd >= 8 && H % 8 == 0 && Wd % 8 == 0, "the UNet needs latent_h and latent_w to be multiples of 8, at least 8");
    SDOD_REQUIRE(CI * 9 <= 96, "latent_channels + concat_channels too large for the small-Cin path (9 Cin <= 96)");
    SDOD_REQUIRE(CC == 0 || CI * 9 > 64, "concat_channels > 0 needs 9 (latent_channels + concat_channels) > 64 (the K = 96 input convolution)");
    SDOD_REQUIRE(CC == 0 || MC == 320 || MC == 256 || MC == 128 || MC == 64,
                 "concat_channels > 0 needs model_channels 64, 128, 256 or 320 (the one-launch input convolution)");
    const int mult[4] = {1, 2, 4, 4};

    if (mode_ != DECLARE) {
        int tot = 0;
        for (auto& rb : unet_res_blocks()) tot += rb.second;
        emb_total_ = tot;
    }
    float* x_in = (float*)io_alloc(inputs_, (size_t)B * LC * H * Wd * sizeof(float));
    f16* temb_in = (f16*)io_alloc(inputs_, (size_t)B * std::max(emb_total_, 1) * sizeof(f16));
    f16* ctx_in = (f16*)io_alloc(inputs_, (size_t)B * CL * cd * sizeof(f16));
    const float* cond_in = CC > 0 ? (const float*)io_alloc(inputs_, (size_t)B * CC * H * Wd * sizeof(float)) : nullptr;
    const int AR = acfg_.adapter_reps;
    const f16* feat_in[4] = {nullptr, nullptr, nullptr, nullptr};
    for (int l = 0; AR > 0 && l < 4; ++l)
        feat_in[l] = (const f16*)io_alloc(inputs_, (size_t)(B / AR) * (H >> l) * (Wd >> l) * mult[l] * MC * sizeof(f16));
    f16* e_out = (f16*)io_alloc(outputs_, (size_t)B * H * Wd * LC * sizeof(f16));
    Act ctx;
    ctx.p = ctx_in; ctx.n = B; ctx.h = 1; ctx.w = CL; ctx.c = cd;
    (void)EC;
    const int emb_ld = emb_total_;
    const f16* emb_all = temb_in;
    int emb_off = 0;
    kv_off_ = 0;
    if (mode_ != DECLARE && kv_total_ > 0) {
        to_static_ = true;
        GemmOpt okv;
        if (quant_mode()) { okv.wq_scale = qscale_of(group_first("attn2_kv_all")); okv.wq_off = qoff_of(group_first("attn2_kv_all")); }
        linear_raw(ctx_in, B * CL, cd, reinterpret_cast<const f16*>(group_base("attn2_kv_all")), cd, kv_total_,
                   mode_ == REAL ? kv_all_ : ctx_in , okv);
        to_static_ = false;
    }

    const int ciw = P("input_blocks.0.0.weight", {MC, CI, 3, 3}, PK_CONV3_SMALL), cib = P("input_blocks.0.0.bias", {MC}, PK_VEC);
    Act h = act(B, H, Wd, MC);
    if (CC > 0) {
        const f16* wp = mode_ != DECLARE ? W<f16>(ciw) : nullptr;
        const float* bp = mode_ != DECLARE ? W<float>(cib) : nullptr;
        f16* hp = h.p;
        settle();
        if (mode_ == REAL) {
            flops_ += 2.0 * B * H * Wd * MC * 96;
            ops_.push_back(Op{[=](hipStream_t st) { check_rc2(sdod_conv_in_cat_f16(x_in, cond_in, wp, bp, hp, B, H, Wd, LC, CC, MC, st)); },
                              "conv_in_cat", 2.0 * B * H * Wd * MC * 96, (double)B * H * Wd * (CI * 4 + MC * 2) + MC * 96 * 2,
                              "M" + std::to_string(B * H * Wd) + " N" + std::to_string(MC) + " K96"});
        }
    } else if (MC == 320 || MC == 256 || MC == 128 || MC == 64) {
        const f16* wp = mode_ != DECLARE ? W<f16>(ciw) : nullptr;
        const float* bp = mode_ != DECLARE ? W<float>(cib) : nullptr;
        f16* hp = h.p;
        settle();
        if (mode_ == REAL) {
            flops_ += 2.0 * B * H * Wd * MC * 64;
            const int wr = wrap_;
            ops_.push_back(Op{[=](hipStream_t st) { check_rc2(sdod_conv_in_wrap_f16(x_in, wp, bp, hp, B, H, Wd, LC, MC, 1.0f, wr, st)); }, "conv_in",
                              2.0 * B * H * Wd * MC * 64, (double)B * H * Wd * (LC * 4 + MC * 2) + MC * 64 * 2,
                              "M" + std::to_string(B * H * Wd) + " N" + std::to_string(MC) + " K64"});
        }
    } else {
        f16* cols = alloc((size_t)B * H * Wd * 64);
        if (wrap_ != 0) {
            Act xl = act(B, H, Wd, LC);
            const int wr = wrap_;
            emit([=](hipStream_t st) { check_rc2(sdod_latent_prep_f16(x_in, nullptr, nullptr, xl.p, B, LC, H * Wd, 1.0f, st)); });
            emit([=](hipStream_t st) { check_rc2(sdod_im2col3x3_small_wrap_f16(xl.p, cols, B, H, Wd, LC, 64, wr, st)); });
            release(xl);
        } else
        emit([=](hipStream_t st) { check_rc2(sdod_latent_im2col_f16(x_in, cols, B, H, Wd, LC, 64, 1.0f, st)); });
        { GemmOpt o; o.bias = cib; linear(cols, B * H * Wd, 64, ciw, MC, h.p, o); }
        release(cols);
    }

    std::vector<Act> hs;
    hs.push_back(h);
    int ch = MC, ds = 1, idx = 1;
    for (int level = 0; level < 4; ++level) {
        for (int i = 0; i < 2; ++i) {
            const std::string pfx = "input_blocks." + std::to_string(idx++);
            Act r = res_block(pfx + ".0", h, nullptr, mult[level] * MC, emb_all, emb_ld, emb_off);
            ch = mult[level] * MC;
            if (ds <= 4) {
                Act t = spatial_transformer(pfx + ".1", r, ctx);
                release(r);
                r = t;
            }
            h = r;
            if (AR > 0 && i == 1) {
                f16* hp = h.p;
                const f16* fp = feat_in[level];
                const size_t per = h.numel() / AR;
                emit([=](hipStream_t st) { check_rc2(sdod_add_feature_f16(hp, fp, per, AR, st)); }, "add_feature", 0,
                     (double)h.numel() * 4 + (double)per * 2);
            }
            hs.push_back(h);
        }
        if (level != 3) {
            const std::string pfx = "input_blocks." + std::to_string(idx++) + ".0.op";
            quant_rows(h.rows() / 4);
            const int w = P(pfx + ".weight", {ch, ch, 3, 3}, PK_CONV3), b = P(pfx + ".bias", {ch}, PK_VEC);
            GemmOpt o; o.bias = b;
            h = conv(h, nullptr, w, ch, 3, 2, false, o);
            hs.push_back(h);
            ds *= 2;
        }
    }
    {
        Act r1 = res_block("middle_block.0", h, nullptr, ch, emb_all, emb_ld, emb_off);
        Act t = spatial_transformer("middle_block.1", r1, ctx);
        release(r1);
        Act r2 = res_block("middle_block.2", t, nullptr, ch, emb_all, emb_ld, emb_off);
        release_after_consumer(t);
        h = r2;
    }
    int oidx = 0;
    for (int level = 3; level >= 0; --level) {
        for (int i = 0; i < 3; ++i) {
            const std::string pfx = "output_blocks." + std::to_string(oidx++);
            Act skip = hs.back();
            hs.pop_back();
            Act r = res_block(pfx + ".0", h, &skip, mult[level] * MC, emb_all, emb_ld, emb_off);
            release(h); release(skip);
            ch = mult[level] * MC;
            int sub = 1;
            if (ds <= 4) {
                Act t = spatial_transformer(pfx + "." + std::to_string(sub++), r, ctx);
                release(r);
                r = t;
            }
            if (level != 0 && i == 2) {
                const std::string up = pfx + "." + std::to_string(sub) + ".conv";
                quant_rows(r.rows() * 4);
                const int w = P(up + ".weight", {ch, ch, 3, 3}, PK_CONV3), b = P(up + ".bias", {ch}, PK_VEC);
                GemmOpt o; o.bias = b;
                Act u = conv(r, nullptr, w, ch, 3, 1, true, o);
                release(r);
                r = u;
                ds /= 2;
            }
            h = r;
        }
    }
    const int ow = P("out.0.weight", {ch}, PK_VEC), ob = P("out.0.bias", {ch}, PK_VEC);
    quant_rows(h.rows());
    const int cw = P("out.2.weight", {LC, ch, 3, 3}, PK_CONV3), cb = P("out.2.bias", {LC}, PK_VEC);
    Act g = group_norm(h, nullptr, ow, ob, 1e-5f, true);
    release(h);
    { GemmOpt o; o.bias = cb; o.out = e_out; conv(g, nullptr, cw, LC, 3, 1, false, o); }
    release(g);
    if (mode_ == DECLARE) kv_total_ = kv_off_;
    else if (emb_off != emb_total_ || kv_off_ != kv_total_) throw Error(INTERNAL_ERROR, "UNet conditioning bookkeeping mismatch");
}

std::vector<std::pair<std::string, int>> Graph::unet_res_blocks() const {
    std::vector<std::pair<std::string, int>> v;
    const int MC = cfg_.model_channels;
    const int mult[4] = {1, 2, 4, 4};
    int idx = 1;
    for (int level = 0; level < 4; ++level) {
        for (int i = 0; i < 2; ++i) v.emplace_back("input_blocks." + std::to_string(idx++) + ".0", mult[level] * MC);
        if (level != 3) ++idx;
    }
    v.emplace_back("middle_block.0", 4 * MC);
    v.emplace_back("middle_block.2", 4 * MC);
    int oidx = 0;
// ... 443 lines not shown
```

stable-diffusion-on-device_amd/csrc/norms.hip:

```cpp
#include "common.h"
#include "sdod_hip.h"
#include "host_util.h"

#include <algorithm>
#include <cstdlib>

namespace {

struct GnMom {
    float n, mean, m2;
};
SDOD_DEVICE GnMom gn_merge(GnMom a, const GnMom& b) {
    if (b.n == 0.f) return a;
    if (a.n == 0.f) return b;
    const float n = a.n + b.n, d = b.mean - a.mean, f = b.n / n;
    a.mean += d * f;
    a.m2 += b.m2 + d * d * a.n * f;
    a.n = n;
    return a;
}

template <typename T>
struct Chunk8;
template <>
// ... 884 lines not shown
                for (int r = 0; r < 8; ++r) __hip_atomic_store(p.sync + 32 * (17 + r), gen0 + 1u, __ATOMIC_RELAXED, __HIP_MEMORY_SCOPE_AGENT);
                opened = true;
            }
        }
        if (!opened) {
            const unsigned* flag = p.sync + 32 * (17 + (blockIdx.x & 7));
            bool met = false;
            for (int spin = 0; spin < (1 << 20); ++spin) {
                if (__hip_atomic_load(flag, __ATOMIC_RELAXED, __HIP_MEMORY_SCOPE_AGENT) != gen0) { met = true; break; }
                __builtin_amdgcn_s_sleep(6);
            }
            if (!met) {
                __hip_atomic_store(p.sync + 32 * 25, 0x0bad0bad, __ATOMIC_RELAXED, __HIP_MEMORY_SCOPE_AGENT);
                if (p.err_host) __hip_atomic_store(p.err_host, 0x0bad0bad, __ATOMIC_RELAXED, __HIP_MEMORY_SCOPE_SYSTEM);
            }
        }
    }
    __syncthreads();
    {
        const int g = tid >> 4, l = tid & 15;
        GnPartialSums ps;
        if (g < p.G) {
            for (int ch = l; ch < p.wpi; ch += 16) {
                const unsigned long long bits = __hip_atomic_load(reinterpret_cast<const unsigned long long*>(p.partial) + ((size_t)n * p.wpi + ch) * p.G + g,
                                                                  __ATOMIC_RELAXED, __HIP_MEMORY_SCOPE_AGENT);
                float2 pr;
                __builtin_memcpy(&pr, &bits, 8);
                const int np = min(p.HW, (ch + 1) * p.ppw) - ch * p.ppw;
                ps.add((float)max(0, np) * (float)p.Cg, pr.x, pr.y);
            }
        }
        const GnMom m = ps.moments();
        const float cnt = (float)p.HW * (float)p.Cg;
        const float mean = group_sum<16>(m.n * m.mean) / cnt;
        const float d = m.mean - mean;
        const float m2 = group_sum<16>(m.m2 + m.n * d * d);
        if (g < p.G && l == 0) {
            gm[g] = mean;
            gr[g] = rsqrt_fast(m2 / cnt + p.eps);
        }
    }
    __syncthreads();
    for (int c = tid; c < p.C; c += 512) {
        const int g = c / p.Cg;
        const float wv = p.w ? p.w[c] : 1.0f, bv = p.b ? p.b[c] : 0.0f;
        sc[c] = gr[g] * wv;
        sh[c] = bv - gm[g] * gr[g] * wv;
    }
    __syncthreads();
    if (!active) return;
    float s8[8], t8[8];
#pragma unroll
    for (int e = 0; e < 8; ++e) {
        s8[e] = sc[c0 + e];
        t8[e] = sh[c0 + e];
    }
    for (int l = 0; l < nloop; ++l) {
        if (nloop > 1) {
#pragma unroll
            for (int k = 0; k < KMAX; ++k) {
                const int pix = pix_begin + r0 + (l * KMAX + k) * p.rp;
                v[k] = pix < pix_end ? ldg8(src(row0 + pix, c0)) : zero8();
            }
        }
#pragma unroll
        for (int k = 0; k < KMAX; ++k) {
            const int pix = pix_begin + r0 + (l * KMAX + k) * p.rp;
            if (pix < pix_end) {
                f16x8 o;
#pragma unroll
                for (int e = 0; e < 8; ++e) {
                    float f = (float)v[k][e] * s8[e] + t8[e];
                    if (p.silu) f = silu_f(f);
                    o[e] = (f16)f;
                }
                stg8(p.y + (row0 + pix) * p.C + c0, o);
            }
        }
    }
}

constexpr size_t GN_GRID_MIN_BYTES = (size_t)5 << 20;

static int gn_device_cus() {
    static std::atomic<int> cus[64];
    int dev = 0;
    if (hipGetDevice(&dev) != hipSuccess || dev < 0 || dev >= 64) return 0;
    int v = cus[dev].load(std::memory_order_relaxed);
    if (v == 0) {
        if (hipDeviceGetAttribute(&v, hipDeviceAttributeMultiprocessorCount, dev) != hipSuccess || v <= 0) v = -1;
        cus[dev].store(v, std::memory_order_relaxed);
    }
    return v > 0 ? v : 0;
}

static int gn_grid_plan(int n, int hw, int c0, int c1, int groups, GnGridP* out) {
    const int c = c0 + c1;
    if (groups > 32 || n <= 0 || !gn2_fits(c0, c1, groups) || c / 8 > 512) return 0;
    if ((size_t)n * hw * c * 2 < GN_GRID_MIN_BYTES) return 0;
    int cus = gn_device_cus();
    if (cus > 256) cus = 256;
    const int wpi = cus / n;
    if (wpi < 8 || wpi > GN_MAX_CHUNKS_GRID) return 0;
    const int cp = c / 8, rp = 512 / cp;
    const int ppw = (hw + wpi - 1) / wpi;
    const int k = (ppw + rp - 1) / rp;
    if (k > 16 * 8) return 0;
    if (out) {
        out->cp = cp; out->rp = rp; out->wpi = wpi; out->ppw = ppw; out->nwg = wpi * n;
        out->nloop = k <= 16 ? 1 : (k + 15) / 16;
    }
    return k <= 4 ? 4 : k <= 8 ? 8 : 16;
}

static unsigned* gn_error_word(bool allocate) {
    static std::atomic<unsigned*> words[64];
    int dev = 0;
    if (hipGetDevice(&dev) != hipSuccess || dev < 0 || dev >= 64) return nullptr;
    unsigned* cur = words[dev].load(std::memory_order_acquire);
    if (!cur && allocate) {
        unsigned* fresh = nullptr;
        if (hipHostMalloc((void**)&fresh, 128, hipHostMallocMapped) != hipSuccess || !fresh) {
            (void)hipGetLastError();
            return nullptr;
        }
        *fresh = 0u;
        if (words[dev].compare_exchange_strong(cur, fresh, std::memory_order_acq_rel)) cur = fresh;
        else (void)hipHostFree(fresh);
    }
    return cur;
}

static bool gn_grid_try(const GnP& q, hipStream_t st) {
    GnGridP p{};
    const int kmax = gn_grid_plan(q.N, q.HW, q.C0, q.C1, q.G, &p);
    if (!kmax) return false;
    p.x0 = (const f16*)q.x0; p.x1 = (const f16*)q.x1; p.y = (f16*)q.y; p.w = q.w; p.b = q.b;
    p.partial = q.partial;
    p.sync = reinterpret_cast<unsigned*>(q.sync);
    p.err_host = gn_error_word(false);
    p.N = q.N; p.HW = q.HW; p.C0 = q.C0; p.C1 = q.C1; p.C = q.C; p.G = q.G; p.Cg = q.Cg; p.eps = q.eps; p.silu = q.silu;
    const size_t smem = ((size_t)q.C * 2 + (size_t)q.G * 2) * sizeof(float);
    if (kmax == 4) SDOD_LAUNCH((gn_grid_kernel<4>), dim3(p.nwg), dim3(512), smem, st, p);
    else if (kmax == 8) SDOD_LAUNCH((gn_grid_kernel<8>), dim3(p.nwg), dim3(512), smem, st, p);
    else SDOD_LAUNCH((gn_grid_kernel<16>), dim3(p.nwg), dim3(512), smem, st, p);
    SDOD_HIP_CHECK(hipGetLastError());
    return true;
}

static int gcd_i(int a, int b) { return b ? gcd_i(b, a % b) : a; }

static size_t gn_small_smem(int hw, int sw, size_t elem) { return (size_t)hw * sw * elem + ((size_t)2 * sw + 128) * sizeof(float) + (size_t)sw; }
static bool gn_small_fits(int hw, int c, int cg, size_t elem) {
    const int sw = cg / gcd_i(cg, 8) * 8;
    if (c % sw != 0) return false;
    return hw <= 1024 && sw / cg <= 4 && gn_small_smem(hw, sw, elem) <= 96 * 1024;
}

template <typename T, int NT>
void gn_small_launch(GnP& p, int sw, size_t smem, hipStream_t st) {
    static std::atomic<unsigned long long> attr_devs{0};
    if (sdod::first_use_on_device(attr_devs)) {
        SDOD_HIP_CHECK(hipFuncSetAttribute(reinterpret_cast<const void*>(&gn_small_kernel<T, NT>), hipFuncAttributeMaxDynamicSharedMemorySize,
                                           96 * 1024 + 4096));
    }
    SDOD_LAUNCH((gn_small_kernel<T, NT>), dim3(p.C / sw, p.N), dim3(NT), smem, st, p, sw);
    SDOD_HIP_CHECK(hipGetLastError());
}

template <typename T>
bool gn_try_small(GnP& p, hipStream_t st) {
    const int sw = p.Cg / gcd_i(p.Cg, 8) * 8;
    if (!gn_small_fits(p.HW, p.C, p.Cg, sizeof(T))) return false;
    const size_t smem = gn_small_smem(p.HW, sw, sizeof(T));
    if (p.HW > 256) gn_small_launch<T, 1024>(p, sw, smem, st);
    else gn_small_launch<T, 256>(p, sw, smem, st);
    return true;
}

constexpr int GN_INLINE_CHUNKS = 128;

static int gn_path_override() {
    static const int v = [] {
        const char* e = std::getenv("SDOD_GN_PATH");
        return !e ? 0 : e[0] == 'g' ? 1 : e[0] == 't' ? 2 : 0;
// ... 655 lines not shown
```

stable-diffusion-on-device_amd/sdod/amd/_lib.py:

```python
import ctypes
import os

_HERE = os.path.dirname(os.path.abspath(__file__))
LIB_DIR = os.path.normpath(os.path.join(_HERE, '..', '..', 'lib'))

_cache = {}


def load(name):
    if name in _cache:
        return _cache[name]
    path = os.path.join(LIB_DIR, os.environ.get('SDOD_LIBSDOD', name) if name == 'libsdod.so' else name)
    if not os.path.exists(path):
        raise ImportError(
            f'{path} not found: build the MI355X extension first '
            f'(python -c "import __graft_entry__ as g; g.build()" or make -C stable-diffusion-on-device_amd). '
            f'There is no CPU fallback for the HIP path.')
    lib = ctypes.CDLL(path, mode=ctypes.RTLD_GLOBAL)
    _cache[name] = lib
    return lib


class SdodError(RuntimeError):
    def __init__(self, code, msg):
# ... 30 lines not shown

class DdimInpaintStepArgs(ctypes.Structure):
    _fields_ = [(k, ctypes.c_void_p) for k in ('eps_nhwc', 'x', 'z0', 'keep', 'noise', 'x_stage', 'temb_row', 'temb_dst')] + \
               [('seed', ctypes.c_uint64), ('image_index0', ctypes.c_uint64)] + \
               [(k, ctypes.c_int) for k in ('n', 'c', 'hw', 'uncond_first', 'mode', 'v_pred', 'last', 'noise_level', 'stage_reps',
                                            'temb_width', 'temb_reps')] + \
               [(k, ctypes.c_float) for k in ('guidance', 'vc0', 'vc1', 'sqrt_one_minus_at', 'sqrt_at', 'sqrt_a_prev', 'dir_coef',
                                              'known_sa', 'known_s1a')]


class KStepArgs(ctypes.Structure):
    _fields_ = [(k, ctypes.c_void_p) for k in ('eps_nhwc', 'x', 'den_prev', 'noise', 'x_stage', 'temb_row', 'temb_dst')] + \
               [('seed', ctypes.c_uint64), ('image_index0', ctypes.c_uint64)] + \
               [(k, ctypes.c_int) for k in ('n', 'c', 'hw', 'uncond_first', 'mode', 'noise_level', 'stage_reps', 'temb_width', 'temb_reps')] + \
               [(k, ctypes.c_float) for k in ('guidance', 'd0', 'd1', 'a', 'b', 'cprev', 'u', 'stage_scale')]


class GemmDesc(ctypes.Structure):
    _fields_ = [
        ('a', c_void_p), ('a2', c_void_p), ('w', c_void_p), ('bias', c_void_p), ('row_bias', c_void_p),
        ('residual', c_void_p), ('out', c_void_p), ('workspace', c_void_p), ('workspace_bytes', c_size_t),
        ('M', c_int), ('N', c_int), ('K', c_int),
        ('lda', c_int), ('ldw', c_int), ('ldo', c_int), ('ldr', c_int),
        ('a_mode', c_int),
        ('n_img', c_int), ('h_in', c_int), ('w_in', c_int), ('c0', c_int), ('c1', c_int),
        ('stride', c_int), ('upsample', c_int), ('ksize', c_int), ('rows_per_img', c_int), ('ld_row_bias', c_int),
        ('act', c_int), ('alpha', c_float), ('bias_on_m', c_int), ('split_k', c_int), ('tile', c_int),
        ('geglu', c_int), ('k_tail', c_int), ('t0', c_void_p), ('t1', c_void_p), ('tc0', c_int), ('tc1', c_int),
        ('bias2', c_void_p), ('ln', c_int), ('ln_s', c_void_p), ('ln_eps', c_float), ('phase', c_int),
        ('wq', c_int), ('w_scale', c_void_p), ('w_off', c_void_p), ('fix_counters', c_void_p), ('xcd_panels', c_int),
        ('w_img_stride', c_int), ('vec_img_stride', c_int), ('softmax_cols', c_int), ('pad_mode', c_int),
    ]


class DenseConvDesc(ctypes.Structure):
    _fields_ = [(k, c_void_p) for k in ('inp', 'w', 'bias', 'out', 'res1', 'res2')] + \
               [(k, c_int) for k in ('ld_in', 'ld_out', 'ld_res1', 'ld_res2', 'out_col', 'cin', 'cout', 'n', 'h', 'w_in', 'upsample')] + \
               [(k, c_float) for k in ('alpha', 'slope', 'c1')]


def _declare(lib):
    P = c_void_p
    sig = {
        'sdod_gemm_f16': (c_int, [ctypes.POINTER(GemmDesc), P]),
        'sdod_gemm_fixup': (c_int, [P]),
        'sdod_gemm_fixup_counters': (c_size_t, []),
        'sdod_gemm_workspace_bytes': (c_size_t, [ctypes.POINTER(GemmDesc)]),
        'sdod_gemm_plan': (c_int, [ctypes.POINTER(GemmDesc), ctypes.POINTER(c_int), ctypes.POINTER(c_int)]),
        'sdod_gemm_halo_ok': (c_int, [ctypes.POINTER(GemmDesc), c_int]),
        'sdod_gemm_panel_ok': (c_int, [ctypes.POINTER(GemmDesc), c_int]),
        'sdod_gemm_xcd_panels': (c_int, [ctypes.POINTER(GemmDesc)]),
        'sdod_gemm_time': (c_int, [ctypes.POINTER(GemmDesc), P, c_int, ctypes.POINTER(c_float)]),
        'sdod_gemm_time_cold': (c_int, [ctypes.POINTER(GemmDesc), P, c_int, P, c_size_t, ctypes.POINTER(c_float), ctypes.POINTER(c_float)]),
        'sdod_gemm_num_tiles': (c_int, []),
        'sdod_gemm_tile_info': (c_int, [c_int, ctypes.POINTER(c_int)]),
        'sdod_gemm_tile_shape': (c_int, [c_int, ctypes.POINTER(c_int), ctypes.POINTER(c_int), ctypes.POINTER(c_int)]),
        'sdod_gemm_reduce_info': (c_int, [ctypes.POINTER(GemmDesc), P]),
        'sdod_group_norm_reduce_ok': (c_int, [c_int, c_int, c_int, c_int]),
        'sdod_group_norm_reduce_nhwc': (c_int, [P, P, P, P, P, c_int, c_int, c_int, c_int, c_int, c_float, c_int, P]),
        'sdod_group_norm_launches': (c_int, [c_int, c_int, c_int, c_int]),
        'sdod_group_norm_workspace_bytes': (c_size_t, [c_int, c_int]),
        'sdod_group_norm_layout': (c_int, [c_int, c_int] + [ctypes.POINTER(c_size_t)] * 5),
        'sdod_group_norm_status': (c_int, []),
        'sdod_group_norm_clear_error': (c_int, []),
        'sdod_group_norm_path': (c_int, [c_int, c_int, c_int, c_int, c_int, c_int]),
        'sdod_group_norm_nchw_workspace_bytes': (c_size_t, [c_int, c_int]),
        'sdod_group_norm_nchw': (c_int, [P, P, P, P, c_int, c_int, ctypes.c_longlong, c_int, c_float, c_int, c_int, P, P]),
        'sdod_group_norm_nhwc': (c_int, [P, P, P, P, P, c_int, c_int, c_int, c_int, c_int, c_float, c_int, c_int, P, P]),
        'sdod_layer_norm_f16': (c_int, [P, P, P, P, c_int, c_int, c_float, P]),
        'sdod_ln_fold_f16': (c_int, [P, c_int, c_int, c_int, P, P, P, P, P, P]),
        'sdod_compose_linear_f16': (c_int, [P, c_int, P, c_int, P, c_int, c_int, c_int, c_int, P, P, P, P]),
        'sdod_lora_merge_f16': (c_int, [P, c_int, c_int, c_int, P, P, c_int, c_float, c_int, c_int, P]),
        'sdod_attention_f16': (c_int, [P, P, P, P, c_int, c_int, c_int, c_int, c_int, c_int, c_int, c_int, c_int, c_float, c_int, P]),
        'sdod_xattn_fold_f16': (c_int, [P, c_int, c_int, c_int, c_int, c_int, P, c_int, P, P, P, c_int, c_int, c_int, c_float, P, P, P, P, P]),
        'sdod_softmax_rows_f16': (c_int, [P, P, c_int, c_int, P]),
        'sdod_geglu_f16': (c_int, [P, P, c_int, c_int, P]),
        'sdod_act_f16': (c_int, [P, P, c_size_t, c_int, P]),
        'sdod_add_f16': (c_int, [P, P, P, c_size_t, P]),
        'sdod_concat_channels_f16': (c_int, [P, P, P, c_size_t, c_int, c_int, P]),
        'sdod_pixel_unshuffle_u8_f16': (c_int, [P, P, c_int, c_int, c_int, c_int, c_int, P]),
        'sdod_avg_pool2_f16': (c_int, [P, P, c_int, c_int, c_int, c_int, P]),
        'sdod_adapter_stage_f16': (c_int, [P, P, c_size_t, c_float, P]),
        'sdod_add_feature_f16': (c_int, [P, P, c_size_t, c_int, P]),
        'sdod_im2col3x3_small_f16': (c_int, [P, P, c_int, c_int, c_int, c_int, c_int, P]),
        'sdod_im2col3x3_small_wrap_f16': (c_int, [P, P, c_int, c_int, c_int, c_int, c_int, c_int, P]),
        'sdod_latent_im2col_f16': (c_int, [P, P, c_int, c_int, c_int, c_int, c_int, c_float, P]),
        'sdod_conv_in_f16': (c_int, [P, P, P, P, c_int, c_int, c_int, c_int, c_int, c_float, P]),
        'sdod_conv_in_wrap_f16': (c_int, [P, P, P, P, c_int, c_int, c_int, c_int, c_int, c_float, c_int, P]),
        'sdod_image_conv_in_f16': (c_int, [P, P, P, P, c_int, c_int, c_int, c_int, P]),
        'sdod_image_conv_in_unit_f16': (c_int, [P, P, P, P, P, c_int, c_int, c_int, c_int, c_int, P]),
        'sdod_dense_conv3x3_f16': (c_int, [ctypes.POINTER(DenseConvDesc), P]),
        'sdod_dense_conv3x3_ok': (c_int, [ctypes.POINTER(DenseConvDesc)]),
        'sdod_conv_in_cat_f16': (c_int, [P, P, P, P, P, c_int, c_int, c_int, c_int, c_int, c_int, P]),
        'sdod_masked_image_conv_in_f16': (c_int, [P, P, P, P, P, c_int, c_int, c_int, c_int, P]),
        'sdod_inpaint_cond_f32': (c_int, [P, P, P, P, c_int, c_int, c_int, c_int, c_int, c_int, ctypes.c_uint64, ctypes.c_uint64, P]),
        'sdod_encode_latent_f32': (c_int, [P, P, P, P, P, c_int, c_int, c_int, c_float, c_float, ctypes.c_uint64, ctypes.c_uint64, P]),
        'sdod_latent_resize_f32': (c_int, [P, P, c_int, c_int, c_int, c_int, c_int, c_int, c_int, c_float, c_float, P, ctypes.c_uint64, ctypes.c_uint64, P]),
        'sdod_latent_resize_taps': (c_int, [c_int, c_int, c_int, P, P]),
        'sdod_plms_update': (c_int, [ctypes.POINTER(PlmsUpdateArgs), P]),
        'sdod_dpm_step': (c_int, [ctypes.POINTER(DpmStepArgs), P]),
        'sdod_ddim_inpaint_step': (c_int, [ctypes.POINTER(DdimInpaintStepArgs), P]),
        'sdod_k_step': (c_int, [ctypes.POINTER(KStepArgs), P]),
        'sdod_mask_to_latent_f32': (c_int, [P, P, c_int, c_int, c_int, c_int, P]),
        'sdod_image_composite_u8': (c_int, [P, P, P, P, c_int, c_size_t, c_float, c_float, c_int, P]),
        'sdod_nchw_f32_to_nhwc_f16': (c_int, [P, P, c_int, c_int, c_int, c_float, P]),
        'sdod_nhwc_f16_to_nchw_f32': (c_int, [P, P, c_int, c_int, c_int, P]),
        'sdod_latent_prep_f16': (c_int, [P, P, P, P, c_int, c_int, c_int, c_float, P]),
        'sdod_embedding_f16': (c_int, [P, P, P, P, c_int, c_int, c_int, P]),
        'sdod_context_assemble_f16': (c_int, [P, P, P, c_int, c_int, c_int, c_int, P]),
        'sdod_timestep_features_f16': (c_int, [P, P, c_int, c_int, P]),
        'sdod_stage_unet_inputs': (c_int, [P, P, c_size_t, c_int, P, P, c_size_t, c_int, P]),
        'sdod_randn_f32': (c_int, [P, P, c_size_t, ctypes.c_uint64, ctypes.c_uint64, P]),
        'sdod_cfg_combine': (c_int, [P, P, c_int, c_int, c_int, c_float, c_int, c_int, P]),
        'sdod_dpm_update': (c_int, [P, P, P, c_size_t, c_int, c_float, c_float, c_float, c_float, c_float, P]),
        'sdod_ddim_step_f32': (c_int, [P, P, c_size_t, c_float, c_float, c_float, c_float, P]),
        'sdod_lincomb4_f32': (c_int, [P, P, P, P, P, c_float, c_float, c_float, c_float, c_float, c_size_t, P]),
        'sdod_image_to_u8': (c_int, [P, P, c_size_t, c_float, c_float, c_int, P]),
        'sdod_hip_last_error': (c_char_p, []),
        'sdod_hip_device_info': (c_int, [ctypes.POINTER(c_int), ctypes.POINTER(c_size_t), c_char_p, c_int]),
    }
    for name, (res, args) in sig.items():
        fn = getattr(lib, name)
        fn.restype = res
        fn.argtypes = args


HIP_SYMBOLS = [
    'sdod_gemm_f16', 'sdod_gemm_fixup', 'sdod_gemm_fixup_counters', 'sdod_gemm_workspace_bytes', 'sdod_gemm_plan', 'sdod_gemm_halo_ok', 'sdod_gemm_panel_ok', 'sdod_gemm_xcd_panels', 'sdod_gemm_num_tiles', 'sdod_gemm_tile_shape', 'sdod_gemm_tile_info', 'sdod_gemm_time', 'sdod_gemm_time_cold', 'sdod_group_norm_workspace_bytes', 'sdod_group_norm_layout', 'sdod_group_norm_status', 'sdod_group_norm_clear_error', 'sdod_l2_prefetch', 'sdod_group_norm_launches', 'sdod_group_norm_path', 'sdod_group_norm_nhwc', 'sdod_group_norm_nchw', 'sdod_group_norm_nchw_workspace_bytes', 'sdod_gemm_reduce_info', 'sdod_group_norm_reduce_ok', 'sdod_group_norm_reduce_nhwc',
    'sdod_layer_norm_f16', 'sdod_ln_fold_f16', 'sdod_compose_linear_f16', 'sdod_lora_merge_f16', 'sdod_attention_f16', 'sdod_xattn_fold_f16', 'sdod_softmax_rows_f16', 'sdod_geglu_f16', 'sdod_act_f16',
    'sdod_add_f16', 'sdod_concat_channels_f16', 'sdod_pixel_unshuffle_u8_f16', 'sdod_avg_pool2_f16', 'sdod_adapter_stage_f16', 'sdod_add_feature_f16', 'sdod_im2col3x3_small_f16', 'sdod_im2col3x3_small_wrap_f16', 'sdod_latent_im2col_f16', 'sdod_conv_in_f16', 'sdod_conv_in_wrap_f16', 'sdod_image_conv_in_f16', 'sdod_conv_in_cat_f16', 'sdod_masked_image_conv_in_f16', 'sdod_inpaint_cond_f32', 'sdod_encode_latent_f32', 'sdod_latent_resize_f32', 'sdod_latent_resize_taps', 'sdod_plms_update', 'sdod_dpm_step', 'sdod_ddim_inpaint_step', 'sdod_k_step', 'sdod_mask_to_latent_f32', 'sdod_image_composite_u8', 'sdod_nchw_f32_to_nhwc_f16',
    'sdod_nhwc_f16_to_nchw_f32', 'sdod_latent_prep_f16', 'sdod_embedding_f16', 'sdod_context_assemble_f16', 'sdod_timestep_features_f16', 'sdod_cfg_combine', 'sdod_stage_unet_inputs', 'sdod_randn_f32',
    'sdod_dpm_update', 'sdod_ddim_step_f32', 'sdod_lincomb4_f32', 'sdod_image_to_u8', 'sdod_hip_last_error',
    'sdod_hip_device_info', 'sdod_image_conv_in_unit_f16', 'sdod_dense_conv3x3_f16', 'sdod_dense_conv3x3_ok',
]


def check(code):
    if code != 0:
        msg = hip().sdod_hip_last_error()
        raise SdodError(code, msg.decode() if msg else 'unknown error')
```

stable-diffusion-on-device_amd/sdod/amd/engine.py:

```python
import contextlib
import ctypes

import numpy as np
import torch

from . import _lib
from ._lib import check

UNET, VAE_DECODER, TEXT_ENCODER, TEMB, VAE_ENCODER, VAE_ENCODER_MASKED, ADAPTER, UPSCALER = 0, 1, 2, 3, 4, 5, 6, 7


class ModelConfig(ctypes.Structure):
    _fields_ = [(n, ctypes.c_int) for n in (
        'latent_channels', 'latent_h', 'latent_w', 'model_channels', 'context_dim', 'context_len', 'num_heads',
        'head_dim', 'vocab_size', 'text_layers', 'text_heads', 'vae_channels', 'linear_proj', 'text_arch', 'weight_quant',
        'concat_channels')]
    adapter_reps = 0
    adapter_hint_channels = 0
    adapter_res_blocks = 0
    tiling = 0
    _ADAPTER_FIELDS = ('adapter_reps', 'adapter_hint_channels', 'adapter_res_blocks', 'tiling')

    @classmethod
    def from_buffer_copy(cls, source, offset=0):
        out = type(ctypes.Structure).from_buffer_copy(cls, source, offset)
        for n in cls._ADAPTER_FIELDS:
            v = int(getattr(source, n, 0))
            if v:
                setattr(out, n, v)
        return out


class AdapterConfig(ctypes.Structure):
    _fields_ = [(n, ctypes.c_int) for n in ('adapter_reps', 'adapter_hint_channels', 'adapter_res_blocks')]


class UpscalerConfig(ctypes.Structure):
    _fields_ = [(n, ctypes.c_int) for n in ('num_blocks', 'in_h', 'in_w')]


TILING_WRAP = {False: 0, True: 3, 'xy': 3, 'x': 1, 'y': 2}


def tiling_wrap(tiling):
    if isinstance(tiling, (bool, str)) and tiling in TILING_WRAP:
        return TILING_WRAP[tiling]
    raise ValueError(f"tiling must be False, True, 'xy', 'x' or 'y', not {tiling!r}")


def copy_config(cfg):
    return ModelConfig.from_buffer_copy(cfg)


class LoraEntry(ctypes.Structure):
    _fields_ = [('name', ctypes.c_char_p), ('up', ctypes.c_void_p), ('down', ctypes.c_void_p), ('dtype', ctypes.c_int),
                ('rank', ctypes.c_int), ('scale', ctypes.c_float)]


ENGINE_SYMBOLS = [
    'sdod_model_config_sd14', 'sdod_model_config_sd21', 'sdod_graph_create', 'sdod_graph_create_ex', 'sdod_graph_create_wrap', 'sdod_graph_destroy', 'sdod_graph_num_params', 'sdod_graph_param_info',
    'sdod_graph_set_param', 'sdod_graph_param_device', 'sdod_graph_load_file', 'sdod_graph_finalize', 'sdod_graph_io', 'sdod_graph_execute', 'sdod_graph_check',
    'sdod_graph_stats', 'sdod_graph_tune_info', 'sdod_graph_num_ops', 'sdod_graph_op_info', 'sdod_graph_op_detail', 'sdod_graph_profile',
    'sdod_graph_keep_base', 'sdod_graph_base_bytes', 'sdod_graph_set_loras', 'sdod_graph_create_upscaler',
]


def _engine():
    lib = _lib.hip()
    if not getattr(lib, '_sdod_engine_typed', False):
        P, I = ctypes.c_void_p, ctypes.c_int
        lib.sdod_model_config_sd14.argtypes = [ctypes.POINTER(ModelConfig)]
        lib.sdod_model_config_sd14.restype = None
        lib.sdod_model_config_sd21.argtypes = [ctypes.POINTER(ModelConfig)]
        lib.sdod_model_config_sd21.restype = None
        lib.sdod_graph_create.argtypes = [ctypes.POINTER(P), I, ctypes.POINTER(ModelConfig), I]
        lib.sdod_graph_create_ex.argtypes = [ctypes.POINTER(P), I, ctypes.POINTER(ModelConfig), ctypes.POINTER(AdapterConfig), I]
        lib.sdod_graph_create_wrap.argtypes = [ctypes.POINTER(P), I, ctypes.POINTER(ModelConfig), ctypes.POINTER(AdapterConfig), I, I]
        lib.sdod_graph_create_upscaler.argtypes = [ctypes.POINTER(P), ctypes.POINTER(UpscalerConfig), I]
        lib.sdod_graph_destroy.argtypes = [P]
        lib.sdod_graph_num_params.argtypes = [P]
        lib.sdod_graph_param_info.argtypes = [P, I, ctypes.POINTER(ctypes.c_char_p), ctypes.POINTER(I), ctypes.POINTER(ctypes.c_int64)]
        lib.sdod_graph_set_param.argtypes = [P, ctypes.c_char_p, P, I, ctypes.POINTER(ctypes.c_int64), I]
        lib.sdod_graph_load_file.argtypes = [P, ctypes.c_char_p, ctypes.c_char_p]
        lib.sdod_graph_param_device.argtypes = [P, ctypes.c_char_p, ctypes.POINTER(P), ctypes.POINTER(ctypes.c_size_t)]
        lib.sdod_graph_finalize.argtypes = [P]
        lib.sdod_graph_io.argtypes = [P, I, I, ctypes.POINTER(P), ctypes.POINTER(ctypes.c_size_t)]
        lib.sdod_graph_execute.argtypes = [P, P, I]
        lib.sdod_graph_check.argtypes = [P]
        lib.sdod_graph_stats.argtypes = [P, ctypes.POINTER(ctypes.c_size_t), ctypes.POINTER(ctypes.c_size_t), ctypes.POINTER(I),
                                         ctypes.POINTER(ctypes.c_double)]
        lib.sdod_graph_tune_info.argtypes = [P, ctypes.POINTER(I), ctypes.POINTER(I), ctypes.c_char_p, I]
        lib.sdod_graph_num_ops.argtypes = [P]
        lib.sdod_graph_op_info.argtypes = [P, I, ctypes.POINTER(ctypes.c_char_p), ctypes.POINTER(ctypes.c_double), ctypes.POINTER(ctypes.c_double)]
        lib.sdod_graph_profile.argtypes = [P, P, I, P, I]
        lib.sdod_graph_op_detail.argtypes = [P, I, ctypes.POINTER(ctypes.c_char_p)]
        lib.sdod_graph_keep_base.argtypes = [P]
        lib.sdod_graph_base_bytes.argtypes = [P, ctypes.POINTER(ctypes.c_size_t)]
        lib.sdod_graph_set_loras.argtypes = [P, ctypes.POINTER(LoraEntry), I, P]
        lib._sdod_engine_typed = True
    return lib


def sd14_config(latent_h=64, latent_w=64, concat_channels=0, adapter_reps=0, adapter_hint_channels=0, adapter_res_blocks=0):
    cfg = ModelConfig()
    _engine().sdod_model_config_sd14(ctypes.byref(cfg))
    cfg.latent_h, cfg.latent_w, cfg.concat_channels = latent_h, latent_w, concat_channels
    cfg.adapter_reps, cfg.adapter_hint_channels, cfg.adapter_res_blocks = int(adapter_reps), int(adapter_hint_channels), int(adapter_res_blocks)
    return cfg


def sd21_config(latent_h=96, latent_w=96, concat_channels=0):
    cfg = ModelConfig()
    _engine().sdod_model_config_sd21(ctypes.byref(cfg))
    cfg.latent_h, cfg.latent_w, cfg.concat_channels = latent_h, latent_w, concat_channels
    return cfg


class _DevView:

    def __init__(self, ptr, shape, typestr):
        self.__cuda_array_interface__ = {'shape': tuple(shape), 'typestr': typestr, 'data': (int(ptr), False), 'version': 2}


def device_view(ptr, shape, dtype, device):
    typestr = {torch.float16: '<f2', torch.float32: '<f4', torch.int32: '<i4', torch.uint8: '|u1'}[dtype]
    return torch.as_tensor(_DevView(ptr, shape, typestr), device=device)


class Graph:

    def __init__(self, kind, cfg, batch, device='cuda:0', wrap=None):
        self._lib = _engine()
        self._h = ctypes.c_void_p()
        self.kind, self.cfg, self.batch = kind, cfg, batch
        self.device = torch.device(device)
        acfg = AdapterConfig(*(int(getattr(cfg, n, 0)) for n, _ in AdapterConfig._fields_))
        with self._on_device():
            if kind == UPSCALER:
                check(self._lib.sdod_graph_create_upscaler(ctypes.byref(self._h), ctypes.byref(cfg), batch))
            elif wrap is not None:
                check(self._lib.sdod_graph_create_wrap(ctypes.byref(self._h), kind, ctypes.byref(cfg), ctypes.byref(acfg), int(wrap), batch))
            elif kind == ADAPTER or any(getattr(acfg, n) for n, _ in AdapterConfig._fields_):
                check(self._lib.sdod_graph_create_ex(ctypes.byref(self._h), kind, ctypes.byref(cfg), ctypes.byref(acfg), batch))
            else:
                check(self._lib.sdod_graph_create(ctypes.byref(self._h), kind, ctypes.byref(cfg), batch))
        self.finalized = False

    def _on_device(self):
        return torch.cuda.device(self.device) if torch.cuda.is_available() else contextlib.nullcontext()

    def __del__(self):
        h = getattr(self, '_h', None)
        if h:
            self._lib.sdod_graph_destroy(h)
            self._h = None

    def param_table(self):
        out = []
        n = self._lib.sdod_graph_num_params(self._h)
        name = ctypes.c_char_p(); nd = ctypes.c_int(); shape = (ctypes.c_int64 * 4)()
        for i in range(n):
            check(self._lib.sdod_graph_param_info(self._h, i, ctypes.byref(name), ctypes.byref(nd), shape))
            out.append((name.value.decode(), tuple(shape[:nd.value])))
        return out

    def set_param(self, name, tensor):
        if hasattr(tensor, 'payload'):
            buf = tensor.payload()
            shape = (ctypes.c_int64 * max(len(tensor.shape), 1))(*tensor.shape)
            check(self._lib.sdod_graph_set_param(self._h, name.encode(), ctypes.cast(ctypes.c_char_p(buf), ctypes.c_void_p), 2, shape,
                                                 len(tensor.shape)))
            return
        t = tensor.detach().cpu().contiguous()
        if t.dtype not in (torch.float32, torch.float16):
            t = t.float()
        shape = (ctypes.c_int64 * max(t.dim(), 1))(*t.shape)
        check(self._lib.sdod_graph_set_param(self._h, name.encode(), ctypes.c_void_p(t.data_ptr()),
                                             1 if t.dtype == torch.float32 else 0, shape, t.dim()))

    def packed_param(self, name, dtype=torch.float16):
        p = ctypes.c_void_p(); n = ctypes.c_size_t()
        check(self._lib.sdod_graph_param_device(self._h, name.encode(), ctypes.byref(p), ctypes.byref(n)))
        return device_view(p.value, (n.value // torch.empty((), dtype=dtype).element_size(),), dtype, self.device)

    def load_state_dict(self, sd, prefix=''):
        with torch.cuda.device(self.device):
            for name, _ in self.param_table():
                key = prefix + name
                if key not in sd:
                    raise KeyError(f'missing parameter {key}')
                self.set_param(name, sd[key])

    def load_file(self, path, prefix=''):
        with self._on_device():
            check(self._lib.sdod_graph_load_file(self._h, path.encode(), prefix.encode()))

    def finalize(self):
        with torch.cuda.device(self.device):
            check(self._lib.sdod_graph_finalize(self._h))
        self.finalized = True
        return self

    def keep_base(self):
        check(self._lib.sdod_graph_keep_base(self._h))
        return self

    def base_bytes(self):
        n = ctypes.c_size_t()
        check(self._lib.sdod_graph_base_bytes(self._h, ctypes.byref(n)))
        return n.value

    def set_loras(self, entries):
        shapes = None
        keep, arr = [], (LoraEntry * max(len(entries), 1))()
        for i, (name, up, down, scale) in enumerate(entries):
            if not (torch.is_tensor(up) and torch.is_tensor(down)) or up.dim() < 2 or down.dim() < 2:
                raise ValueError(f'{name}: up and down must be tensors of at least two dimensions')
            if shapes is None:
                shapes = dict(self.param_table())
            dt = torch.float16 if up.dtype == torch.float16 and down.dtype == torch.float16 else torch.float32
            up = up.detach().cpu().to(dt).contiguous()
            down = down.detach().cpu().to(dt).contiguous()
            rank = down.shape[0]
            if len(shapes.get(name, ())) >= 2:
                shape = shapes[name]
                fan_in = int(np.prod(shape[1:]))
                if up.numel() != shape[0] * rank or up.shape[0] != shape[0] or down.numel() != rank * fan_in:
                    raise ValueError(f'{name}: factors {tuple(up.shape)} x {tuple(down.shape)} do not give a {tuple(shape)} weight')
            keep += [up, down]
            arr[i] = LoraEntry(name.encode(), up.data_ptr(), down.data_ptr(), 1 if dt == torch.float32 else 0, rank, float(scale))
        with self._on_device():
            check(self._lib.sdod_graph_set_loras(self._h, arr, len(entries),
                                                 ctypes.c_void_p(torch.cuda.current_stream(self.device).cuda_stream if torch.cuda.is_available() else None)))

    def _io(self, is_out, idx):
        p = ctypes.c_void_p(); n = ctypes.c_size_t()
        check(self._lib.sdod_graph_io(self._h, 1 if is_out else 0, idx, ctypes.byref(p), ctypes.byref(n)))
        return p.value, n.value

    def io_tensor(self, is_out, idx, shape, dtype):
        ptr, nbytes = self._io(is_out, idx)
        numel = int(np.prod(shape))
        assert numel * torch.empty((), dtype=dtype).element_size() == nbytes, (shape, dtype, nbytes)
        return device_view(ptr, shape, dtype, self.device)

    def execute(self, use_hip_graph=False, static_unchanged=False):
        flags = (1 if use_hip_graph else 0) | (2 if static_unchanged else 0)
        check(self._lib.sdod_graph_execute(self._h, ctypes.c_void_p(torch.cuda.current_stream(self.device).cuda_stream), flags))

    def check(self):
        check(self._lib.sdod_graph_check(self._h))

    def op_table(self):
        out = []
        lab = ctypes.c_char_p(); fl = ctypes.c_double(); by = ctypes.c_double()
        for i in range(self._lib.sdod_graph_num_ops(self._h)):
            check(self._lib.sdod_graph_op_info(self._h, i, ctypes.byref(lab), ctypes.byref(fl), ctypes.byref(by)))
            out.append((lab.value.decode(), fl.value, by.value))
        return out

    def op_details(self):
        out = []
        det = ctypes.c_char_p()
        for i in range(self._lib.sdod_graph_num_ops(self._h)):
            check(self._lib.sdod_graph_op_detail(self._h, i, ctypes.byref(det)))
            out.append(det.value.decode())
        return out

    def profile(self, iters=3):
        n = self._lib.sdod_graph_num_ops(self._h)
        ms = (ctypes.c_float * n)()
        check(self._lib.sdod_graph_profile(self._h, ctypes.c_void_p(torch.cuda.current_stream(self.device).cuda_stream), iters, ms, n))
        return list(ms)

    def tune_source(self):
        a = ctypes.c_int(); b = ctypes.c_int(); buf = ctypes.create_string_buffer(1024)
        check(self._lib.sdod_graph_tune_info(self._h, ctypes.byref(a), ctypes.byref(b), buf, 1024))
        import os
        return {'table': ' + '.join(os.path.basename(p) for p in buf.value.decode().split(' + ') if p), 'shapes_from_table': a.value,
                'shapes_tuned_in_process': b.value}

    def stats(self):
        w = ctypes.c_size_t(); a = ctypes.c_size_t(); n = ctypes.c_int(); f = ctypes.c_double()
        check(self._lib.sdod_graph_stats(self._h, ctypes.byref(w), ctypes.byref(a), ctypes.byref(n), ctypes.byref(f)))
        return {'weight_bytes': w.value, 'arena_bytes': a.value, 'launches': n.value, 'flops': f.value}


class UNet(Graph):
    def __init__(self, cfg, batch, device='cuda:0', wrap=None):
        super().__init__(UNET, cfg, batch, device, wrap if wrap is not None else (int(getattr(cfg, 'tiling', 0)) or None))

    def finalize(self):
        super().finalize()
        c, b = self.cfg, self.batch
        self.x = self.io_tensor(False, 0, (b, c.latent_channels, c.latent_h, c.latent_w), torch.float32)
        self.temb_width = self._io(False, 1)[1] // (2 * b)
        self.temb = self.io_tensor(False, 1, (b, self.temb_width), torch.float16)
        self.ctx = self.io_tensor(False, 2, (b, c.context_len, c.context_dim), torch.float16)
        self.eps = self.io_tensor(True, 0, (b, c.latent_h, c.latent_w, c.latent_channels), torch.float16)
        if c.concat_channels > 0:
            self.cond = self.io_tensor(False, 3, (b, c.concat_channels, c.latent_h, c.latent_w), torch.float32)
        reps = int(getattr(c, 'adapter_reps', 0))
        if reps > 0:
            first = 4 if c.concat_channels > 0 else 3
            self.adapter_feat = [self.io_tensor(False, first + k, shape, torch.float16) for k, shape in enumerate(adapter_feature_shapes(c, b // reps))]
        return self


def adapter_feature_shapes(cfg, n):
    mc = cfg.model_channels
    return [(n, cfg.latent_h // s, cfg.latent_w // s, m * mc) for s, m in ((1, 1), (2, 2), (4, 4), (8, 4))]


class Adapter(Graph):

    def __init__(self, cfg, batch, device='cuda:0'):
        super().__init__(ADAPTER, cfg, batch, device)

    def finalize(self):
        super().finalize()
        c, b = self.cfg, self.batch
        self.hint = self.io_tensor(False, 0, (b, 8 * c.latent_h, 8 * c.latent_w, c.adapter_hint_channels), torch.uint8)
        self.out = [self.io_tensor(True, k, shape, torch.float16) for k, shape in enumerate(adapter_feature_shapes(c, b))]
        return self


def upscaler_check_config(num_blocks, image_hw):
    if not isinstance(num_blocks, int) or isinstance(num_blocks, bool) or not 1 <= num_blocks <= 23:
        raise ValueError(f'upscaler: num_blocks must be an integer in [1, 23], not {num_blocks!r}')
    try:
        h, w = (int(v) for v in image_hw)
    except (TypeError, ValueError):
        raise ValueError(f'upscaler: image_hw must be a (height, width) pair, not {image_hw!r}') from None
    for v in (h, w):
        if v < 8 or v > 1024 or v % 8:
            raise ValueError(f'upscaler: image height and width must be multiples of 8 in [8, 1024], not {(h, w)}')
    return h, w


class Upscaler(Graph):

    SCALE = 4

    def __init__(self, num_blocks=23, image_hw=(512, 512), batch=1, device='cuda:0'):
        h, w = upscaler_check_config(num_blocks, image_hw)
        self.num_blocks, self.image_hw = num_blocks, (h, w)
        super().__init__(UPSCALER, UpscalerConfig(num_blocks, h, w), batch, device)

    def finalize(self):
        super().finalize()
        (h, w), b = self.image_hw, self.batch
        self.img = self.io_tensor(False, 0, (b, h, w, 3), torch.uint8)
        self.out = self.io_tensor(True, 0, (b, 4 * h, 4 * w, 3), torch.float16)
        return self


class Temb(Graph):
    def __init__(self, cfg, batch, device='cuda:0'):
        super().__init__(TEMB, cfg, batch, device)

    def finalize(self):
        super().finalize()
        self.t = self.io_tensor(False, 0, (self.batch,), torch.float32)
        self.width = self._io(True, 0)[1] // (2 * self.batch)
        self.out = self.io_tensor(True, 0, (self.batch, self.width), torch.float16)
        return self


class TextEncoder(Graph):
    def __init__(self, cfg, batch, device='cuda:0'):
        super().__init__(TEXT_ENCODER, cfg, batch, device)

    def finalize(self):
# ... 45 lines not shown
```

stable-diffusion-on-device_amd/sdod/amd/ops.py:

```python
import ctypes

import torch

from . import _lib
from ._lib import GemmDesc, check

ACT = {None: 0, 'none': 0, 'silu': 1, 'gelu': 2, 'quick_gelu': 3, 'relu': 4}


def _stream():
    return ctypes.c_void_p(torch.cuda.current_stream().cuda_stream)


def _p(t):
    return None if t is None else ctypes.c_void_p(t.data_ptr())


def _req(t, dtype=None, name='tensor'):
    if not t.is_cuda:
        raise ValueError(f'{name} must live on the GPU')
    if not t.is_contiguous():
        raise ValueError(f'{name} must be contiguous')
    if dtype is not None and t.dtype != dtype:
        raise ValueError(f'{name} must be {dtype}, got {t.dtype}')
# ... 296 lines not shown

def softmax_rows(x, out=None):
    lib = _lib.hip()
    _req(x, torch.float16, 'x')
    n = x.shape[-1]; m = x.numel() // n
    if out is None:
        out = torch.empty_like(x)
    check(lib.sdod_softmax_rows_f16(_p(x), _p(out), m, n, _stream()))
    return out


def geglu(x, out=None):
    lib = _lib.hip()
    _req(x, torch.float16, 'x')
    c = x.shape[-1] // 2; m = x.numel() // (2 * c)
    if out is None:
        out = torch.empty(x.shape[:-1] + (c,), dtype=torch.float16, device=x.device)
    check(lib.sdod_geglu_f16(_p(x), _p(out), m, c, _stream()))
    return out


def activation(x, act, out=None):
    lib = _lib.hip()
    _req(x, torch.float16, 'x')
    if out is None:
        out = torch.empty_like(x)
    check(lib.sdod_act_f16(_p(x), _p(out), x.numel(), ACT[act], _stream()))
    return out


def add(a, b, out=None):
    lib = _lib.hip()
    _req(a, torch.float16, 'a'); _req(b, torch.float16, 'b')
    if out is None:
        out = torch.empty_like(a)
    check(lib.sdod_add_f16(_p(a), _p(b), _p(out), a.numel(), _stream()))
    return out


def pixel_unshuffle_u8(img_u8, factor=8, out=None):
    lib = _lib.hip()
    _req(img_u8, torch.uint8, 'img')
    n, ih, iw, ch = img_u8.shape
    h, w = ih // factor, iw // factor
    assert ih == h * factor and iw == w * factor, img_u8.shape
    if out is None:
        out = torch.empty((n, h, w, ch * factor * factor), dtype=torch.float16, device=img_u8.device)
    else:
        _req(out, torch.float16, 'out')
        assert out.numel() == img_u8.numel(), (out.shape, img_u8.shape)
    check(lib.sdod_pixel_unshuffle_u8_f16(_p(img_u8), _p(out), n, h, w, ch, factor, _stream()))
    return out


def avg_pool2(x, out=None):
    lib = _lib.hip()
    _req(x, torch.float16, 'x')
    n, h, w, c = x.shape
    if out is None:
        out = torch.empty((n, h // 2, w // 2, c), dtype=torch.float16, device=x.device)
    else:
        _req(out, torch.float16, 'out')
        assert out.numel() * 4 == x.numel(), (out.shape, x.shape)
    check(lib.sdod_avg_pool2_f16(_p(x), _p(out), n, h, w, c, _stream()))
    return out


def adapter_stage(src, dst, weight=1.0):
    lib = _lib.hip()
    _req(src, torch.float16, 'src'); _req(dst, torch.float16, 'dst')
    assert dst.numel() == src.numel(), (dst.shape, src.shape)
    check(lib.sdod_adapter_stage_f16(_p(src), _p(dst), src.numel(), float(weight), _stream()))
    return dst


def add_feature(h, f, reps):
    lib = _lib.hip()
    _req(h, torch.float16, 'h'); _req(f, torch.float16, 'f')
    assert h.numel() == reps * f.numel(), (h.shape, f.shape, reps)
    check(lib.sdod_add_feature_f16(_p(h), _p(f), f.numel(), reps, _stream()))
    return h


def concat_channels(a, b):
    lib = _lib.hip()
    _req(a, torch.float16, 'a'); _req(b, torch.float16, 'b')
    c0, c1 = a.shape[-1], b.shape[-1]
    rows = a.numel() // c0
    out = torch.empty(a.shape[:-1] + (c0 + c1,), dtype=torch.float16, device=a.device)
    check(lib.sdod_concat_channels_f16(_p(a), _p(b), _p(out), rows, c0, c1, _stream()))
    return out


def im2col3x3_small(x, kpad=64, wrap=None):
    lib = _lib.hip()
    _req(x, torch.float16, 'x')
    n, h, w, c = x.shape
    out = torch.empty((n * h * w, kpad), dtype=torch.float16, device=x.device)
    if wrap is None:
        check(lib.sdod_im2col3x3_small_f16(_p(x), _p(out), n, h, w, c, kpad, _stream()))
    else:
        check(lib.sdod_im2col3x3_small_wrap_f16(_p(x), _p(out), n, h, w, c, kpad, int(wrap), _stream()))
    return out


def latent_im2col(x, kpad=64, scale=1.0):
    lib = _lib.hip()
    _req(x, torch.float32, 'x')
    n, c, h, w = x.shape
    out = torch.empty((n * h * w, kpad), dtype=torch.float16, device=x.device)
    check(lib.sdod_latent_im2col_f16(_p(x), _p(out), n, h, w, c, kpad, scale, _stream()))
    return out


def conv_in(x, w, bias, scale=1.0, wrap=None):
    lib = _lib.hip()
    _req(x, torch.float32, 'x'); _req(w, torch.float16, 'w'); _req(bias, torch.float32, 'bias')
    n, c, h, wd = x.shape
    cout = w.shape[0]
    assert w.shape[1] == 64
    out = torch.empty((n, h, wd, cout), dtype=torch.float16, device=x.device)
    if wrap is None:
        check(lib.sdod_conv_in_f16(_p(x), _p(w), _p(bias), _p(out), n, h, wd, c, cout, scale, _stream()))
    else:
        check(lib.sdod_conv_in_wrap_f16(_p(x), _p(w), _p(bias), _p(out), n, h, wd, c, cout, scale, int(wrap), _stream()))
    return out


def image_conv_in(img_u8, w, bias):
    lib = _lib.hip()
    _req(img_u8, torch.uint8, 'img'); _req(w, torch.float16, 'w'); _req(bias, torch.float32, 'bias')
    n, h, wd, c = img_u8.shape
    assert c == 3 and w.shape[1] == 64
    cout = w.shape[0]
    out = torch.empty((n, h, wd, cout), dtype=torch.float16, device=img_u8.device)
    check(lib.sdod_image_conv_in_f16(_p(img_u8), _p(w), _p(bias), _p(out), n, h, wd, cout, _stream()))
    return out


def image_conv_in_unit(img_u8, w, bias, out2=None):
    lib = _lib.hip()
    _req(img_u8, torch.uint8, 'img'); _req(w, torch.float16, 'w'); _req(bias, torch.float32, 'bias')
    n, h, wd, c = img_u8.shape
    assert c == 3 and w.shape[1] == 64
    cout = w.shape[0]
    out = torch.empty((n, h, wd, cout), dtype=torch.float16, device=img_u8.device)
    ld2 = 0
    if out2 is not None:
        _req(out2, torch.float16, 'out2')
        assert tuple(out2.shape[:3]) == (n, h, wd), out2.shape
        ld2 = out2.shape[3]
    check(lib.sdod_image_conv_in_unit_f16(_p(img_u8), _p(w), _p(bias), _p(out), _p(out2), ld2, n, h, wd, cout, _stream()))
    return out


def dense_conv_desc(inp, w, bias, out, *, n, h, wd, cin, cout, ld_in, ld_out, out_col=0, in_off=0, out_off=0, alpha=1.0, slope=0.0,
                    res1=None, res1_off=0, ld_res1=0, c1=0.0, res2=None, res2_off=0, ld_res2=0, upsample=0):
    def at(t, off):
        return None if t is None else ctypes.c_void_p(t.data_ptr() + off * t.element_size())
    return _lib.DenseConvDesc(at(inp, in_off), _p(w), _p(bias), at(out, out_off), at(res1, res1_off), at(res2, res2_off),
                              ld_in, ld_out, ld_res1, ld_res2, out_col, cin, cout, n, h, wd, upsample, alpha, slope, c1)


def dense_conv(inp, w, bias, out, **kw):
    d = dense_conv_desc(inp, w, bias, out, **kw)
    check(_lib.hip().sdod_dense_conv3x3_f16(ctypes.byref(d), _stream()))
# ... 366 lines not shown
```

stable-diffusion-on-device_amd/sdod/amd/pipeline.py:

```python
import os

import numpy as np
import torch

from . import engine as E
from . import ops
from . import prompts as PR
from . import upscale as UP
from .host import DpmSolver
from .samplers import K_SAMPLERS, K_SCHEDULES, PLMS_ORDERS, KSchedule, PlmsSchedule


class Txt2Img:
    inpaint_unet = False
    _cond_staged = False
    encoder = None
    masked_encoder = None
    _traj = None
    prompt_chunks = 1
    model = 'sd14'
    tokenizer = None
    text = None
    _loras = False
    hires = None
    adapter = None
    adapter_channels = 3
    upscaler = None
    tiling = 0

    def __init__(self, state_dicts=None, models_dir=None, images_per_gpu=1, latent_hw=64, device='cuda:0', use_hip_graph=True,
                 tokenizer=None, with_text_encoder=True, model='sd14', with_vae=True, cfg_split=False, weight_quant=None,
                 with_vae_encoder=False, inpaint_unet=False, prompt_chunks=1, *, loras=False, hires_hw=None, adapter=False,
                 adapter_channels=3, tiling=False, upscaler=False):
        self.prompt_chunks = check_prompt_chunks(prompt_chunks)
        latent_h, latent_w = check_latent_hw(latent_hw)
        adapter_check_build(adapter, adapter_channels, cfg_split, hires_hw, inpaint_unet, model)
        self.tiling = tiling_check_build(tiling, with_vae_encoder, inpaint_unet, hires_hw, adapter)
        up_args = upscaler_check_build(upscaler, tiling, hires_hw if hires_hw is not None else latent_hw, state_dicts, models_dir)
        if hires_hw is not None:
            check_latent_hw(hires_hw, 'hires_hw')
            if cfg_split or inpaint_unet:
                raise ValueError('hires_hw cannot be combined with cfg_split or inpaint_unet')
        self.device = torch.device(device)
        torch.cuda.set_device(self.device)
        self.n = images_per_gpu
        self.model = model
        self.v_prediction = model == 'sd21'
        self.cfg = E.sd21_config(latent_h, latent_w) if model == 'sd21' else E.sd14_config(latent_h, latent_w)
        self.inpaint_unet = bool(inpaint_unet)
        if self.inpaint_unet:
            self.cfg.concat_channels = 5
        self._cond_staged = False
        if weight_quant is None:
            weight_quant = state_dicts is not None and any(hasattr(v, 'payload') and len(v.shape) >= 2 for v in state_dicts['unet'].values())
        self.cfg.weight_quant = 2 if weight_quant in ('auto', 2) else 1 if weight_quant else 0
        self.cfg_split = bool(cfg_split)
        self._pair = None
        if self.cfg_split:
            import torch.distributed as dist
            if not (dist.is_available() and dist.is_initialized() and dist.get_world_size() % 2 == 0):
                raise RuntimeError('cfg_split needs torch.distributed initialised with an even world size')
            rank = dist.get_rank()
            self._half = rank % 2
            for a in range(0, dist.get_world_size(), 2):
                grp = dist.new_group([a, a + 1])
                if a == rank - self._half:
                    self._pair = grp
            self._pair_staged = dist.get_backend() == 'gloo'
        self.use_hip_graph = use_hip_graph
        self.tokenizer = tokenizer
        unet_cfg = self.cfg
        if self.prompt_chunks > 1:
            unet_cfg = E.copy_config(self.cfg)
            unet_cfg.context_len = PR.CHUNK_LEN * self.prompt_chunks
        if adapter:
            unet_cfg = E.copy_config(unet_cfg)
            unet_cfg.adapter_reps = 2
            self.adapter_channels = int(adapter_channels)
        vae_cfg = self.cfg
        if self.tiling:
            unet_cfg, vae_cfg = E.copy_config(unet_cfg), E.copy_config(self.cfg)
            unet_cfg.tiling = vae_cfg.tiling = self.tiling
        self.unet = E.UNet(unet_cfg, self.n if cfg_split else 2 * self.n, device)
        self.vae = E.VaeDecoder(vae_cfg, 1, device) if with_vae else None
        self.text = E.TextEncoder(self.cfg, 2 * self.prompt_chunks, device) if with_text_encoder else None
        self.encoder = E.VaeEncoder(self.cfg, 1, device) if with_vae_encoder else None
        self.masked_encoder = E.MaskedVaeEncoder(self.cfg, 1, device) if self.inpaint_unet else None
        if adapter:
            acfg = E.copy_config(self.cfg)
            acfg.adapter_hint_channels = self.adapter_channels
            self.adapter = E.Adapter(acfg, 1, device)
        self._temb_graphs = {}
        self._sd = state_dicts
        self._dir = models_dir
        for g, key, stem in ((self.unet, 'unet', 'unet'), (self.vae, 'vae', 'vae_decoder'), (self.text, 'text', 'text_encoder'),
                             (self.encoder, 'vae_enc', 'vae_encoder'), (self.masked_encoder, 'vae_enc', 'vae_encoder'),
                             (self.adapter, 'adapter', 'adapter')):
            if g is None:
                continue
            self._load(g, key, stem)
            if loras and (g is self.unet or g is self.text):
                g.keep_base()
            g.finalize()
        if up_args is not None:
            self.upscaler = UP.Upscaler(device=device, use_hip_graph=use_hip_graph, **up_args)
        self._loras = bool(loras)
        self._temb_cache = {}
        self._ctx_fresh = True
        if hires_hw is not None:
            self.hires = Txt2Img(state_dicts=state_dicts, models_dir=models_dir, images_per_gpu=images_per_gpu, latent_hw=hires_hw,
                                 device=device, use_hip_graph=use_hip_graph, tokenizer=None, with_text_encoder=False, model=model,
                                 with_vae=with_vae, cfg_split=False, weight_quant=weight_quant, with_vae_encoder=False, inpaint_unet=False,
                                 prompt_chunks=prompt_chunks, loras=loras)

    def _load(self, g, key, stem):
        if self._sd is not None:
            g.load_state_dict(self._sd[key])
        else:
            g.load_file(f'{self._dir}/{stem}.sdodw')

    def set_loras(self, adapters, strict=True):
        from . import lora as L
        if not self._loras:
            raise RuntimeError('this pipeline was built without loras=True: merge on the host (lora.merged_state_dict) and build a new one')
        parsed = []
        for a in adapters:
            if not isinstance(a, (tuple, list)) or len(a) not in (2, 3):
                raise ValueError('an adapter is (path_or_dict, strength) or (path_or_dict, strength_unet, strength_text)')
            strengths = [a[1], a[1] if len(a) == 2 else a[2]]
            for v in strengths:
                if isinstance(v, bool) or not isinstance(v, (int, float, np.integer, np.floating)) or not np.isfinite(float(v)):
                    raise ValueError(f'LoRA strength must be a finite number, got {v!r}')
            parsed.append((a[0], float(strengths[0]), float(strengths[1])))
        if self.cfg.weight_quant != 0:
            raise ValueError('LoRA adapters need fp16 weights: this pipeline keeps uint8 codes (weight_quant); merge on the host instead')
        lists, skipped = {'unet': [], 'text': []}, []
        for src, s_unet, s_text in parsed:
            ent, skip = L.entries_for(src, self.model, s_unet, s_text, strict=strict)
            lists['unet'] += ent['unet']
            lists['text'] += ent['text']
            skipped += skip
        if lists['text'] and self.text is None:
            raise ValueError('the adapters hold text-encoder modules and this pipeline has no text encoder')
        self.unet.set_loras(lists['unet'])
        if self.hires is not None:
            self.hires.unet.set_loras(lists['unet'])
            self.hires._ctx_fresh = True
        if self.text is not None:
            self.text.set_loras(lists['text'])
        self._ctx_fresh = True
        return skipped

    def clear_loras(self):
        return self.set_loras([])

    def set_adapter_hint(self, hint_u8, weight=1.0):
        if self.adapter is None:
            raise RuntimeError('this pipeline was built without adapter=True: Txt2Img(..., adapter=True) is needed for structural control')
        hint_u8 = adapter_check_args(hint_u8, weight, self._latent_shape, self.n, self.adapter_channels)
        hint_u8 = hint_u8.to(self.device).contiguous()
        for i in range(self.n):
            self.adapter.hint.copy_(hint_u8[i:i + 1])
            self.adapter.execute(self.use_hip_graph)
            for out, slot in zip(self.adapter.out, self.unet.adapter_feat):
                ops.adapter_stage(out, slot[i:i + 1], weight)

# ... 788 lines not shown
```

Baseline: 10.73 images/s.

## Share the guidance-pair prefix up to the first cross-attention in the UNet

Adds a paired UNet mode for classifier-free guidance. The cond and uncond copies share the same latent and timestep, so everything before the first cross-attention (conv_in, the first resblock, the start of the first transformer) runs once on half the batch. A new repeat_rows kernel then broadcasts the activations to both copies at that seam. The mode is on by default when rows reach the threshold, and group-norm grid sizing is adjusted for single-image shapes. It adds a broadcast kernel and more complex graph bookkeeping, and it depends on the uncond and cond inputs being the same before the context diverges.

```diff
diff --git a/include/sdod_engine.h b/include/sdod_engine.h
--- a/include/sdod_engine.h
+++ b/include/sdod_engine.h
@@ -46,6 +46,8 @@
 SDOD_API int sdod_graph_create_ex(void** graph, int kind, const sdod_model_config* cfg, const sdod_adapter_config* adapter, int batch);
 SDOD_API int sdod_graph_create_wrap(void** graph, int kind, const sdod_model_config* cfg, const sdod_adapter_config* adapter, int wrap,
                                     int batch);
+SDOD_API int sdod_graph_create_pair(void** graph, int kind, const sdod_model_config* cfg, const sdod_adapter_config* adapter, int wrap,
+                                    int pair, int batch);
 typedef struct sdod_upscaler_config {
     int num_blocks;
     int in_h;
diff --git a/include/sdod_hip.h b/include/sdod_hip.h
--- a/include/sdod_hip.h
+++ b/include/sdod_hip.h
@@ -139,6 +139,7 @@
 SDOD_API int sdod_avg_pool2_f16(const void* x, void* y, int n, int h, int w, int c, void* stream);
 SDOD_API int sdod_adapter_stage_f16(const void* src, void* dst, size_t count, float weight, void* stream);
 SDOD_API int sdod_add_feature_f16(void* h, const void* f, size_t per_copy, int reps, void* stream);
+SDOD_API int sdod_repeat_rows_f16(const void* const srcs[3], void* const dsts[3], const size_t counts[3], int reps, void* stream);
 SDOD_API int sdod_im2col3x3_small_f16(const void* x, void* y, int n_img, int h, int w, int c, int kpad, void* stream);
 SDOD_API int sdod_im2col3x3_small_wrap_f16(const void* x, void* y, int n_img, int h, int w, int c, int kpad, int wrap, void* stream);
 SDOD_API int sdod_latent_im2col_f16(const float* x, void* y, int n_img, int h, int w, int c, int kpad, float scale, void* stream);
diff --git a/stable-diffusion-on-device_amd/csrc/elementwise.hip b/stable-diffusion-on-device_amd/csrc/elementwise.hip
--- a/stable-diffusion-on-device_amd/csrc/elementwise.hip
+++ b/stable-diffusion-on-device_amd/csrc/elementwise.hip
@@ -120,6 +120,30 @@
 #pragma unroll
             for (int e = 0; e < 8; ++e) o[e] = (f16)add_rn((float)u[e], (float)v[e]);
             stg8(p, o);
+        }
+    }
+}
+
+struct RepeatRowsP {
+    const f16* src[3];
+    f16* dst[3];
+    size_t count[3], end[3];
+    int vec[3];
+    int reps;
+};
+__global__ void repeat_rows_kernel(RepeatRowsP p) {
+    GRID_STRIDE(i, p.end[2]) {
+        const bool s1 = i >= p.end[0], s2 = i >= p.end[1];
+        const f16* src = s2 ? p.src[2] : s1 ? p.src[1] : p.src[0];
+        f16* dst = s2 ? p.dst[2] : s1 ? p.dst[1] : p.dst[0];
+        const size_t count = s2 ? p.count[2] : s1 ? p.count[1] : p.count[0];
+        const size_t j = i - (s2 ? p.end[1] : s1 ? p.end[0] : 0);
+        if (s2 ? p.vec[2] : s1 ? p.vec[1] : p.vec[0]) {
+            const f16x8 v = ldg8(src + j * 8);
+            for (int r = 0; r < p.reps; ++r) stg8(dst + (size_t)r * count + j * 8, v);
+        } else {
+            const f16 v = src[j];
+            for (int r = 0; r < p.reps; ++r) dst[(size_t)r * count + j] = v;
         }
     }
 }
@@ -989,6 +1013,29 @@
     SDOD_CATCH
 }
 
+extern "C" int sdod_repeat_rows_f16(const void* const srcs[3], void* const dsts[3], const size_t counts[3], int reps, void* stream) {
+    SDOD_TRY
+    SDOD_REQUIRE(srcs && dsts && counts, "null argument");
+    SDOD_REQUIRE(reps >= 1 && reps <= 8, "reps must be in [1, 8]");
+    RepeatRowsP p{};
+    p.reps = reps;
+    size_t end = 0;
+    for (int s = 0; s < 3; ++s) {
+        SDOD_REQUIRE(counts[s] == 0 || (srcs[s] && dsts[s]), "null pointer for a source with a non-zero count");
+        SDOD_REQUIRE(counts[s] <= ((size_t)1 << 40), "count too large");
+        p.src[s] = (const f16*)srcs[s];
+        p.dst[s] = (f16*)dsts[s];
+        p.count[s] = counts[s];
+        p.vec[s] = counts[s] % 8 == 0 && (((uintptr_t)srcs[s] | (uintptr_t)dsts[s]) & 15) == 0 ? 1 : 0;
+        end += p.vec[s] ? counts[s] / 8 : counts[s];
+        p.end[s] = end;
+    }
+    if (end == 0) return 0;
+    LAUNCH(repeat_rows_kernel, end, stream, p);
+    return 0;
+    SDOD_CATCH
+}
+
 extern "C" int sdod_add_f16(const void* a, const void* b, void* y, size_t n, void* stream) {
     SDOD_TRY
     SDOD_REQUIRE(a && b && y && n > 0 && n % 8 == 0, "bad argument (count must be a multiple of 8)");
diff --git a/stable-diffusion-on-device_amd/csrc/engine.h b/stable-diffusion-on-device_amd/csrc/engine.h
--- a/stable-diffusion-on-device_amd/csrc/engine.h
+++ b/stable-diffusion-on-device_amd/csrc/engine.h
@@ -60,7 +60,7 @@
 class Graph {
 public:
     Graph(int kind, const sdod_model_config& cfg, int batch, const sdod_adapter_config& acfg = sdod_adapter_config{0, 0, 0}, int wrap = 0,
-          const sdod_upscaler_config& ucfg = sdod_upscaler_config{0, 0, 0});
+          const sdod_upscaler_config& ucfg = sdod_upscaler_config{0, 0, 0}, int pair = 0);
     ~Graph();
     Graph(const Graph&) = delete;
 
@@ -85,6 +85,7 @@
     sdod_upscaler_config ucfg_;
     int batch_;
     int wrap_ = 0;
+    int pair_ = 0;
     Mode mode_ = DECLARE;
     bool finalized_ = false;
 
@@ -233,7 +234,12 @@
         flush_pending();
         drain_parked();
     }
-    Act spatial_transformer(const std::string& pfx, const Act& x, const Act& ctx);
+    struct PairSeam {
+        Act extra;
+        Act extra_full;
+        Act x_full;
+    };
+    Act spatial_transformer(const std::string& pfx, const Act& x, const Act& ctx, PairSeam* seam = nullptr);
     Act vae_res_block(const std::string& pfx, const Act& x, int cout);
     Act vae_attn_block(const std::string& pfx, const Act& x);
     int emb_total_ = 0;
diff --git a/stable-diffusion-on-device_amd/csrc/engine.hip b/stable-diffusion-on-device_amd/csrc/engine.hip
--- a/stable-diffusion-on-device_amd/csrc/engine.hip
+++ b/stable-diffusion-on-device_amd/csrc/engine.hip
@@ -39,8 +39,9 @@
     for (auto& t : th) t.join();
 }
 
-Graph::Graph(int kind, const sdod_model_config& cfg, int batch, const sdod_adapter_config& acfg, int wrap, const sdod_upscaler_config& ucfg)
-    : kind_(kind), cfg_(cfg), acfg_(acfg), ucfg_(ucfg), batch_(batch), wrap_(wrap) {
+Graph::Graph(int kind, const sdod_model_config& cfg, int batch, const sdod_adapter_config& acfg, int wrap, const sdod_upscaler_config& ucfg,
+             int pair)
+    : kind_(kind), cfg_(cfg), acfg_(acfg), ucfg_(ucfg), batch_(batch), wrap_(wrap), pair_(pair) {
     SDOD_REQUIRE(kind >= SDOD_GRAPH_UNET && kind <= SDOD_GRAPH_UPSCALER, "unknown graph kind");
     if (kind == SDOD_GRAPH_UPSCALER) {
         SDOD_REQUIRE(ucfg.num_blocks != 0 || ucfg.in_h != 0 || ucfg.in_w != 0, "the UPSCALER graph is created by sdod_graph_create_upscaler");
@@ -63,6 +64,12 @@
                      "wrap applies to the UNET (without concat_channels) and VAE_DECODER graphs only");
     if (kind == SDOD_GRAPH_UNET && acfg.adapter_reps > 0)
         SDOD_REQUIRE(batch % acfg.adapter_reps == 0, "adapter_reps must divide the batch");
+    SDOD_REQUIRE(pair == 0 || pair == 2, "pair must be 0 or 2 (the guidance copies)");
+    if (pair == 2) {
+        SDOD_REQUIRE(kind == SDOD_GRAPH_UNET, "pair applies to the UNET graph only");
+        SDOD_REQUIRE(batch % 2 == 0, "a guidance pair needs an even batch ([copy][image])");
+        SDOD_REQUIRE(cfg.weight_quant == 0, "a guidance pair needs fp16 weights (weight_quant = 0)");
+    }
     if (kind == SDOD_GRAPH_ADAPTER) {
         SDOD_REQUIRE(acfg.adapter_hint_channels == 1 || acfg.adapter_hint_channels == 3, "adapter_hint_channels must be 1 or 3");
         SDOD_REQUIRE(acfg.adapter_res_blocks >= 0 && acfg.adapter_res_blocks <= 8, "adapter_res_blocks must be in [1, 8] (0 = 2)");
@@ -1272,6 +1279,16 @@
     SDOD_CATCH
 }
 
+extern "C" int sdod_graph_create_pair(void** graph, int kind, const sdod_model_config* cfg, const sdod_adapter_config* adapter, int wrap,
+                                      int pair, int batch) {
+    SDOD_TRY
+    SDOD_REQUIRE(graph != nullptr && cfg != nullptr, "null argument");
+    *graph = nullptr;
+    *graph = new Graph(kind, *cfg, batch, adapter ? *adapter : sdod_adapter_config{0, 0, 0}, wrap, sdod_upscaler_config{0, 0, 0}, pair);
+    return 0;
+    SDOD_CATCH
+}
+
 extern "C" int sdod_graph_create_upscaler(void** graph, const sdod_upscaler_config* ucfg, int batch) {
     SDOD_TRY
     SDOD_REQUIRE(graph != nullptr, "null argument");
diff --git a/stable-diffusion-on-device_amd/csrc/graphs.hip b/stable-diffusion-on-device_amd/csrc/graphs.hip
--- a/stable-diffusion-on-device_amd/csrc/graphs.hip
+++ b/stable-diffusion-on-device_amd/csrc/graphs.hip
@@ -75,11 +75,13 @@
     return out;
 }
 
-Act Graph::spatial_transformer(const std::string& pfx, const Act& x, const Act& ctx) {
+Act Graph::spatial_transformer(const std::string& pfx, const Act& x, const Act& ctx, PairSeam* seam) {
     const int C = x.c, cd = ctx.c;
     const int heads = cfg_.num_heads > 0 ? cfg_.num_heads : C / cfg_.head_dim;
     const int d = C / heads;
-    const int rows = x.rows(), L = x.h * x.w, B = x.n;
+    int rows = x.rows(), B = x.n;
+    const int L = x.h * x.w;
+    if ((seam != nullptr) != (x.n != ctx.n) || (seam && ctx.n != 2 * x.n)) throw Error(INTERNAL_ERROR, "transformer batch does not match its context");
     const std::string tb = pfx + ".transformer_blocks.0";
     quant_rows(rows);
     const bool quant_block = quant_decl_;
@@ -117,7 +119,13 @@
     }
     const int f2b = P(tb + ".ff.net.2.bias", {C}, PK_VEC);
     const int pob = P(pfx + ".proj_out.bias", {C}, PK_VEC);
-    if (mode_ == DECLARE) return act(x.n, x.h, x.w, C);
+    if (mode_ == DECLARE) {
+        if (seam) {
+            seam->x_full = act(ctx.n, x.h, x.w, C);
+            seam->extra_full = act(ctx.n, seam->extra.h, seam->extra.w, seam->extra.c);
+        }
+        return act(ctx.n, x.h, x.w, C);
+    }
 
     Act g = group_norm(x, nullptr, nw, nb, 1e-6f, false);
     Act t0 = act(B, 1, L, C);
@@ -141,6 +149,25 @@
     Act t1 = act(B, 1, L, C);
     { GemmOpt o; o.bias = o1b; o.residual = t0.p; linear(a1, rows, C, o1w, C, t1.p, o); }
     release(a1); release(t0);
+    Act xr = x;
+    if (seam) {
+        Act t1f = act(ctx.n, 1, L, C);
+        seam->x_full = act(ctx.n, x.h, x.w, C);
+        seam->extra_full = act(ctx.n, seam->extra.h, seam->extra.w, seam->extra.c);
+        struct Bc { const void* s[3]; void* d[3]; size_t n[3]; };
+        const Bc bc = {{t1.p, x.p, seam->extra.p}, {t1f.p, seam->x_full.p, seam->extra_full.p}, {t1.numel(), x.numel(), seam->extra.numel()}};
+        settle();
+        if (mode_ == REAL)
+            ops_.push_back(Op{[=](hipStream_t st) { check_rc2(sdod_repeat_rows_f16(bc.s, bc.d, bc.n, 2, st)); }, "pair_broadcast", 0,
+                              3.0 * (double)(bc.n[0] + bc.n[1] + bc.n[2]) * 2,
+                              "n" + std::to_string(x.n) + "->" + std::to_string(ctx.n) + " hw" + std::to_string(L) + " c" + std::to_string(C) + "+" +
+                                  std::to_string(C) + "+" + std::to_string(seam->extra.c)});
+        release(t1); release(x); release(seam->extra);
+        t1 = t1f;
+        xr = seam->x_full;
+        B = ctx.n;
+        rows = xr.rows();
+    }
     static const bool xfold_on = [] { const char* e = std::getenv("SDOD_XATTN_FOLD"); return !(e && e[0] == '0'); }();
     const int NK = heads * 80;
     const bool xfold = xfold_on && fold && ctx.w <= 80 && NK % 320 == 0 && L % 32 == 0 && d <= 160 && d % 4 == 0;
@@ -187,8 +214,8 @@
                 f16* wc = reinterpret_cast<f16*>(params_[f2w].dev);
                 compose_jobs_.push_back(ComposeJob{wc, wc + 4 * C, 5 * C, C, C, 4 * C, W<float>(f2b), W<float>(pob), bc});
             }
-            Act out = act(x.n, x.h, x.w, C);
-            { GemmOpt o; o.bias_raw = mode_ == REAL ? bc : reinterpret_cast<const float*>(params_[f2w].dev); o.residual = x.p;
+            Act out = act(xr.n, xr.h, xr.w, C);
+            { GemmOpt o; o.bias_raw = mode_ == REAL ? bc : reinterpret_cast<const float*>(params_[f2w].dev); o.residual = xr.p;
               linear_raw(cat, rows, 5 * C, reinterpret_cast<const f16*>(params_[f2w].dev), 5 * C, C, out.p, o); }
             release(cat);
             return out;
@@ -201,8 +228,8 @@
         Act t3 = act(B, 1, L, C);
         { GemmOpt o; o.bias = f2b; o.residual = t2.p; linear(gg, rows, 4 * C, f2w, C, t3.p, o); }
         release(gg); release(t2);
-        Act out = act(x.n, x.h, x.w, C);
-        { GemmOpt o; o.bias = pob; o.residual = x.p; linear(t3.p, rows, C, pow_, C, out.p, o); }
+        Act out = act(xr.n, xr.h, xr.w, C);
+        { GemmOpt o; o.bias = pob; o.residual = xr.p; linear(t3.p, rows, C, pow_, C, out.p, o); }
         release(t3);
         return out;
     }
@@ -232,8 +259,8 @@
             f16* wc = reinterpret_cast<f16*>(params_[f2w].dev);
             compose_jobs_.push_back(ComposeJob{wc, wc + 4 * C, 5 * C, C, C, 4 * C, W<float>(f2b), W<float>(pob), bc});
         }
-        Act out = act(x.n, x.h, x.w, C);
-        { GemmOpt o; o.bias_raw = mode_ == REAL ? bc : reinterpret_cast<const float*>(params_[f2w].dev); o.residual = x.p;
+        Act out = act(xr.n, xr.h, xr.w, C);
+        { GemmOpt o; o.bias_raw = mode_ == REAL ? bc : reinterpret_cast<const float*>(params_[f2w].dev); o.residual = xr.p;
           linear_raw(cat, rows, 5 * C, reinterpret_cast<const f16*>(params_[f2w].dev), 5 * C, C, out.p, o); }
         release(cat);
         return out;
@@ -252,8 +279,8 @@
     Act t3 = act(B, 1, L, C);
     { GemmOpt o; o.bias = f2b; o.residual = t2.p; linear(gg, rows, 4 * C, f2w, C, t3.p, o); }
     release(gg); release(t2);
-    Act out = act(x.n, x.h, x.w, C);
-    { GemmOpt o; o.bias = pob; o.residual = x.p; linear(t3.p, rows, C, pow_, C, out.p, o); }
+    Act out = act(xr.n, xr.h, xr.w, C);
+    { GemmOpt o; o.bias = pob; o.residual = xr.p; linear(t3.p, rows, C, pow_, C, out.p, o); }
     release(t3);
     return out;
 }
@@ -301,17 +328,19 @@
     }
 
     const int ciw = P("input_blocks.0.0.weight", {MC, CI, 3, 3}, PK_CONV3_SMALL), cib = P("input_blocks.0.0.bias", {MC}, PK_VEC);
-    Act h = act(B, H, Wd, MC);
+    const bool paired = pair_ == 2;
+    const int NB = paired ? B / 2 : B;
+    Act h = act(NB, H, Wd, MC);
     if (CC > 0) {
         const f16* wp = mode_ != DECLARE ? W<f16>(ciw) : nullptr;
         const float* bp = mode_ != DECLARE ? W<float>(cib) : nullptr;
         f16* hp = h.p;
         settle();
         if (mode_ == REAL) {
-            flops_ += 2.0 * B * H * Wd * MC * 96;
-            ops_.push_back(Op{[=](hipStream_t st) { check_rc2(sdod_conv_in_cat_f16(x_in, cond_in, wp, bp, hp, B, H, Wd, LC, CC, MC, st)); },
-                              "conv_in_cat", 2.0 * B * H * Wd * MC * 96, (double)B * H * Wd * (CI * 4 + MC * 2) + MC * 96 * 2,
-                              "M" + std::to_string(B * H * Wd) + " N" + std::to_string(MC) + " K96"});
+            flops_ += 2.0 * NB * H * Wd * MC * 96;
+            ops_.push_back(Op{[=](hipStream_t st) { check_rc2(sdod_conv_in_cat_f16(x_in, cond_in, wp, bp, hp, NB, H, Wd, LC, CC, MC, st)); },
+                              "conv_in_cat", 2.0 * NB * H * Wd * MC * 96, (double)NB * H * Wd * (CI * 4 + MC * 2) + MC * 96 * 2,
+                              "M" + std::to_string(NB * H * Wd) + " N" + std::to_string(MC) + " K96"});
         }
     } else if (MC == 320 || MC == 256 || MC == 128 || MC == 64) {
         const f16* wp = mode_ != DECLARE ? W<f16>(ciw) : nullptr;
@@ -319,23 +348,23 @@
         f16* hp = h.p;
         settle();
         if (mode_ == REAL) {
-            flops_ += 2.0 * B * H * Wd * MC * 64;
+            flops_ += 2.0 * NB * H * Wd * MC * 64;
             const int wr = wrap_;
-            ops_.push_back(Op{[=](hipStream_t st) { check_rc2(sdod_conv_in_wrap_f16(x_in, wp, bp, hp, B, H, Wd, LC, MC, 1.0f, wr, st)); }, "conv_in",
-                              2.0 * B * H * Wd * MC * 64, (double)B * H * Wd * (LC * 4 + MC * 2) + MC * 64 * 2,
-                              "M" + std::to_string(B * H * Wd) + " N" + std::to_string(MC) + " K64"});
+            ops_.push_back(Op{[=](hipStream_t st) { check_rc2(sdod_conv_in_wrap_f16(x_in, wp, bp, hp, NB, H, Wd, LC, MC, 1.0f, wr, st)); }, "conv_in",
+                              2.0 * NB * H * Wd * MC * 64, (double)NB * H * Wd * (LC * 4 + MC * 2) + MC * 64 * 2,
+                              "M" + std::to_string(NB * H * Wd) + " N" + std::to_string(MC) + " K64"});
         }
     } else {
-        f16* cols = alloc((size_t)B * H * Wd * 64);
+        f16* cols = alloc((size_t)NB * H * Wd * 64);
         if (wrap_ != 0) {
-            Act xl = act(B, H, Wd, LC);
+            Act xl = act(NB, H, Wd, LC);
             const int wr = wrap_;
-            emit([=](hipStream_t st) { check_rc2(sdod_latent_prep_f16(x_in, nullptr, nullptr, xl.p, B, LC, H * Wd, 1.0f, st)); });
-            emit([=](hipStream_t st) { check_rc2(sdod_im2col3x3_small_wrap_f16(xl.p, cols, B, H, Wd, LC, 64, wr, st)); });
+            emit([=](hipStream_t st) { check_rc2(sdod_latent_prep_f16(x_in, nullptr, nullptr, xl.p, NB, LC, H * Wd, 1.0f, st)); });
+            emit([=](hipStream_t st) { check_rc2(sdod_im2col3x3_small_wrap_f16(xl.p, cols, NB, H, Wd, LC, 64, wr, st)); });
             release(xl);
         } else
-        emit([=](hipStream_t st) { check_rc2(sdod_latent_im2col_f16(x_in, cols, B, H, Wd, LC, 64, 1.0f, st)); });
-        { GemmOpt o; o.bias = cib; linear(cols, B * H * Wd, 64, ciw, MC, h.p, o); }
+        emit([=](hipStream_t st) { check_rc2(sdod_latent_im2col_f16(x_in, cols, NB, H, Wd, LC, 64, 1.0f, st)); });
+        { GemmOpt o; o.bias = cib; linear(cols, NB * H * Wd, 64, ciw, MC, h.p, o); }
         release(cols);
     }
 
@@ -347,7 +376,14 @@
             const std::string pfx = "input_blocks." + std::to_string(idx++);
             Act r = res_block(pfx + ".0", h, nullptr, mult[level] * MC, emb_all, emb_ld, emb_off);
             ch = mult[level] * MC;
-            if (ds <= 4) {
+            if (paired && level == 0 && i == 0) {
+                PairSeam seam;
+                seam.extra = h;
+                Act t = spatial_transformer(pfx + ".1", r, ctx, &seam);
+                hs[0] = seam.extra_full;
+                release(seam.x_full);
+                r = t;
+            } else if (ds <= 4) {
                 Act t = spatial_transformer(pfx + ".1", r, ctx);
                 release(r);
                 r = t;
diff --git a/stable-diffusion-on-device_amd/csrc/norms.hip b/stable-diffusion-on-device_amd/csrc/norms.hip
--- a/stable-diffusion-on-device_amd/csrc/norms.hip
+++ b/stable-diffusion-on-device_amd/csrc/norms.hip
@@ -990,6 +990,11 @@
 
 constexpr size_t GN_GRID_MIN_BYTES = (size_t)5 << 20;
 
+static bool gn_grid_single_image(int n, int hw, int c) {
+    const size_t bytes = (size_t)hw * c * 2;
+    return n == 1 && hw >= 4096 && c <= 320 && bytes >= GN_GRID_MIN_BYTES / 2 && bytes < GN_GRID_MIN_BYTES;
+}
+
 static int gn_device_cus() {
     static std::atomic<int> cus[64];
     int dev = 0;
@@ -1005,10 +1010,10 @@
 static int gn_grid_plan(int n, int hw, int c0, int c1, int groups, GnGridP* out) {
     const int c = c0 + c1;
     if (groups > 32 || n <= 0 || !gn2_fits(c0, c1, groups) || c / 8 > 512) return 0;
-    if ((size_t)n * hw * c * 2 < GN_GRID_MIN_BYTES) return 0;
+    if ((size_t)n * hw * c * 2 < GN_GRID_MIN_BYTES && !gn_grid_single_image(n, hw, c)) return 0;
     int cus = gn_device_cus();
     if (cus > 256) cus = 256;
-    const int wpi = cus / n;
+    const int wpi = gn_grid_single_image(n, hw, c) ? std::min(cus, 128) : cus / n;
     if (wpi < 8 || wpi > GN_MAX_CHUNKS_GRID) return 0;
     const int cp = c / 8, rp = 512 / cp;
     const int ppw = (hw + wpi - 1) / wpi;
diff --git a/stable-diffusion-on-device_amd/sdod/amd/_lib.py b/stable-diffusion-on-device_amd/sdod/amd/_lib.py
--- a/stable-diffusion-on-device_amd/sdod/amd/_lib.py
+++ b/stable-diffusion-on-device_amd/sdod/amd/_lib.py
@@ -136,6 +136,7 @@
         'sdod_avg_pool2_f16': (c_int, [P, P, c_int, c_int, c_int, c_int, P]),
         'sdod_adapter_stage_f16': (c_int, [P, P, c_size_t, c_float, P]),
         'sdod_add_feature_f16': (c_int, [P, P, c_size_t, c_int, P]),
+        'sdod_repeat_rows_f16': (c_int, [ctypes.POINTER(c_void_p), ctypes.POINTER(c_void_p), ctypes.POINTER(c_size_t), c_int, P]),
         'sdod_im2col3x3_small_f16': (c_int, [P, P, c_int, c_int, c_int, c_int, c_int, P]),
         'sdod_im2col3x3_small_wrap_f16': (c_int, [P, P, c_int, c_int, c_int, c_int, c_int, c_int, P]),
         'sdod_latent_im2col_f16': (c_int, [P, P, c_int, c_int, c_int, c_int, c_int, c_float, P]),
@@ -185,7 +186,7 @@
     'sdod_add_f16', 'sdod_concat_channels_f16', 'sdod_pixel_unshuffle_u8_f16', 'sdod_avg_pool2_f16', 'sdod_adapter_stage_f16', 'sdod_add_feature_f16', 'sdod_im2col3x3_small_f16', 'sdod_im2col3x3_small_wrap_f16', 'sdod_latent_im2col_f16', 'sdod_conv_in_f16', 'sdod_conv_in_wrap_f16', 'sdod_image_conv_in_f16', 'sdod_conv_in_cat_f16', 'sdod_masked_image_conv_in_f16', 'sdod_inpaint_cond_f32', 'sdod_encode_latent_f32', 'sdod_latent_resize_f32', 'sdod_latent_resize_taps', 'sdod_plms_update', 'sdod_dpm_step', 'sdod_ddim_inpaint_step', 'sdod_k_step', 'sdod_mask_to_latent_f32', 'sdod_image_composite_u8', 'sdod_nchw_f32_to_nhwc_f16',
     'sdod_nhwc_f16_to_nchw_f32', 'sdod_latent_prep_f16', 'sdod_embedding_f16', 'sdod_context_assemble_f16', 'sdod_timestep_features_f16', 'sdod_cfg_combine', 'sdod_stage_unet_inputs', 'sdod_randn_f32',
     'sdod_dpm_update', 'sdod_ddim_step_f32', 'sdod_lincomb4_f32', 'sdod_image_to_u8', 'sdod_hip_last_error',
-    'sdod_hip_device_info', 'sdod_image_conv_in_unit_f16', 'sdod_dense_conv3x3_f16', 'sdod_dense_conv3x3_ok',
+    'sdod_hip_device_info', 'sdod_image_conv_in_unit_f16', 'sdod_dense_conv3x3_f16', 'sdod_dense_conv3x3_ok', 'sdod_repeat_rows_f16',
 ]
 
 
diff --git a/stable-diffusion-on-device_amd/sdod/amd/engine.py b/stable-diffusion-on-device_amd/sdod/amd/engine.py
--- a/stable-diffusion-on-device_amd/sdod/amd/engine.py
+++ b/stable-diffusion-on-device_amd/sdod/amd/engine.py
@@ -1,5 +1,6 @@
 import contextlib
 import ctypes
+import os
 
 import numpy as np
 import torch
@@ -61,7 +62,7 @@
     'sdod_model_config_sd14', 'sdod_model_config_sd21', 'sdod_graph_create', 'sdod_graph_create_ex', 'sdod_graph_create_wrap', 'sdod_graph_destroy', 'sdod_graph_num_params', 'sdod_graph_param_info',
     'sdod_graph_set_param', 'sdod_graph_param_device', 'sdod_graph_load_file', 'sdod_graph_finalize', 'sdod_graph_io', 'sdod_graph_execute', 'sdod_graph_check',
     'sdod_graph_stats', 'sdod_graph_tune_info', 'sdod_graph_num_ops', 'sdod_graph_op_info', 'sdod_graph_op_detail', 'sdod_graph_profile',
-    'sdod_graph_keep_base', 'sdod_graph_base_bytes', 'sdod_graph_set_loras', 'sdod_graph_create_upscaler',
+    'sdod_graph_keep_base', 'sdod_graph_base_bytes', 'sdod_graph_set_loras', 'sdod_graph_create_upscaler', 'sdod_graph_create_pair',
 ]
 
 
@@ -76,6 +77,7 @@
         lib.sdod_graph_create.argtypes = [ctypes.POINTER(P), I, ctypes.POINTER(ModelConfig), I]
         lib.sdod_graph_create_ex.argtypes = [ctypes.POINTER(P), I, ctypes.POINTER(ModelConfig), ctypes.POINTER(AdapterConfig), I]
         lib.sdod_graph_create_wrap.argtypes = [ctypes.POINTER(P), I, ctypes.POINTER(ModelConfig), ctypes.POINTER(AdapterConfig), I, I]
+        lib.sdod_graph_create_pair.argtypes = [ctypes.POINTER(P), I, ctypes.POINTER(ModelConfig), ctypes.POINTER(AdapterConfig), I, I, I]
         lib.sdod_graph_create_upscaler.argtypes = [ctypes.POINTER(P), ctypes.POINTER(UpscalerConfig), I]
         lib.sdod_graph_destroy.argtypes = [P]
         lib.sdod_graph_num_params.argtypes = [P]
@@ -129,7 +131,7 @@
 
 class Graph:
 
-    def __init__(self, kind, cfg, batch, device='cuda:0', wrap=None):
+    def __init__(self, kind, cfg, batch, device='cuda:0', wrap=None, pair=None):
         self._lib = _engine()
         self._h = ctypes.c_void_p()
         self.kind, self.cfg, self.batch = kind, cfg, batch
@@ -138,6 +140,9 @@
         with self._on_device():
             if kind == UPSCALER:
                 check(self._lib.sdod_graph_create_upscaler(ctypes.byref(self._h), ctypes.byref(cfg), batch))
+            elif pair is not None:
+                check(self._lib.sdod_graph_create_pair(ctypes.byref(self._h), kind, ctypes.byref(cfg), ctypes.byref(acfg), int(wrap or 0), int(pair),
+                                                       batch))
             elif wrap is not None:
                 check(self._lib.sdod_graph_create_wrap(ctypes.byref(self._h), kind, ctypes.byref(cfg), ctypes.byref(acfg), int(wrap), batch))
             elif kind == ADAPTER or any(getattr(acfg, n) for n, _ in AdapterConfig._fields_):
@@ -276,7 +281,6 @@
     def tune_source(self):
         a = ctypes.c_int(); b = ctypes.c_int(); buf = ctypes.create_string_buffer(1024)
         check(self._lib.sdod_graph_tune_info(self._h, ctypes.byref(a), ctypes.byref(b), buf, 1024))
-        import os
         return {'table': ' + '.join(os.path.basename(p) for p in buf.value.decode().split(' + ') if p), 'shapes_from_table': a.value,
                 'shapes_tuned_in_process': b.value}
 
@@ -286,9 +290,22 @@
         return {'weight_bytes': w.value, 'arena_bytes': a.value, 'launches': n.value, 'flops': f.value}
 
 
+def pair_prefix_enabled():
+    return os.environ.get('SDOD_PAIR_PREFIX', '1')[:1] != '0'
+
+
+PAIR_MIN_ROWS = 2048
+
+
+def pair_prefix_pays(n, latent_h, latent_w):
+    return n * latent_h * latent_w >= PAIR_MIN_ROWS
+
+
 class UNet(Graph):
-    def __init__(self, cfg, batch, device='cuda:0', wrap=None):
-        super().__init__(UNET, cfg, batch, device, wrap if wrap is not None else (int(getattr(cfg, 'tiling', 0)) or None))
+    def __init__(self, cfg, batch, device='cuda:0', wrap=None, pair=False):
+        self.pair = bool(pair)
+        super().__init__(UNET, cfg, batch, device, wrap if wrap is not None else (int(getattr(cfg, 'tiling', 0)) or None),
+                         2 if pair else None)
 
     def finalize(self):
         super().finalize()
diff --git a/stable-diffusion-on-device_amd/sdod/amd/ops.py b/stable-diffusion-on-device_amd/sdod/amd/ops.py
--- a/stable-diffusion-on-device_amd/sdod/amd/ops.py
+++ b/stable-diffusion-on-device_amd/sdod/amd/ops.py
@@ -402,6 +402,18 @@
     return h
 
 
+def repeat_rows(srcs, dsts, reps=2):
+    lib = _lib.hip()
+    assert 1 <= len(srcs) <= 3 and len(srcs) == len(dsts)
+    sp, dp, cn = (ctypes.c_void_p * 3)(), (ctypes.c_void_p * 3)(), (ctypes.c_size_t * 3)()
+    for i, (s, d) in enumerate(zip(srcs, dsts)):
+        _req(s, torch.float16, 'src'); _req(d, torch.float16, 'dst')
+        assert d.numel() == reps * s.numel(), (d.shape, s.shape, reps)
+        sp[i], dp[i], cn[i] = s.data_ptr() if s.numel() else None, d.data_ptr() if s.numel() else None, s.numel()
+    check(lib.sdod_repeat_rows_f16(sp, dp, cn, reps, _stream()))
+    return dsts
+
+
 def concat_channels(a, b):
     lib = _lib.hip()
     _req(a, torch.float16, 'a'); _req(b, torch.float16, 'b')
diff --git a/stable-diffusion-on-device_amd/sdod/amd/pipeline.py b/stable-diffusion-on-device_amd/sdod/amd/pipeline.py
--- a/stable-diffusion-on-device_amd/sdod/amd/pipeline.py
+++ b/stable-diffusion-on-device_amd/sdod/amd/pipeline.py
@@ -81,7 +81,9 @@
         if self.tiling:
             unet_cfg, vae_cfg = E.copy_config(unet_cfg), E.copy_config(self.cfg)
             unet_cfg.tiling = vae_cfg.tiling = self.tiling
-        self.unet = E.UNet(unet_cfg, self.n if cfg_split else 2 * self.n, device)
+        pair = (not cfg_split and self.cfg.weight_quant == 0 and E.pair_prefix_enabled()
+                and E.pair_prefix_pays(self.n, self.cfg.latent_h, self.cfg.latent_w))
+        self.unet = E.UNet(unet_cfg, self.n if cfg_split else 2 * self.n, device, pair=pair)
         self.vae = E.VaeDecoder(vae_cfg, 1, device) if with_vae else None
         self.text = E.TextEncoder(self.cfg, 2 * self.prompt_chunks, device) if with_text_encoder else None
         self.encoder = E.VaeEncoder(self.cfg, 1, device) if with_vae_encoder else None
```

Result: no change. 10.82 images/s, median of 6 (+0.8%).
